# daovietanh190499/3D_Reconstruction

Hardware: AMD Instinct MI355X
Metric: image-pairs matched/sec (higher is better)
Workload: dtype f32 descriptors: int8 MFMA certified filter + f64 re-score; 1 GPU; C3/C4 all-pairs BF-L2 + ratio 0.75: 257 imgs x 4096 kpts x 256-d, exact f32-input semantics (oracle.match.bf_match_exact, bit for bit); pairs=32896, api=dist.match_all_pairs_sharded(exact=True), match_mode=exact-float, parallelism=pairs/1

## Files before the change

### 3d_reconstruction_amd/csrc/match.hip

```cpp
#include "common.h"
#include "fp6_sched.h"
#include <climits>
#include <cstdlib>

namespace sfmhip {

typedef int i32x4 __attribute__((ext_vector_type(4)));
typedef int i32x16 __attribute__((ext_vector_type(16)));

constexpr int kJB = 128;

template <int D>
__device__ __forceinline__ int swz_off(int r, int c) {
    constexpr int CPR = D / 16;
    constexpr int RPB = 256 / D;
    return r * D + ((c ^ ((r / RPB) % CPR)) << 4);
}

__device__ __forceinline__ int max3i(int a, int b, int c) {
    int r;
    asm("v_max3_i32 %0, %1, %2, %3" : "=v"(r) : "v"(a), "v"(b), "v"(c));
    return r;
}
__device__ __forceinline__ int med3i(int a, int b, int c) {
    int r;
    asm("v_med3_i32 %0, %1, %2, %3" : "=v"(r) : "v"(a), "v"(b), "v"(c));
    return r;
}

__global__ void quantize_kernel(const float* __restrict__ in, int64_t total, int d, int m_pad,
                                const int32_t* __restrict__ nk, int mode, int8_t* __restrict__ out) {
    const int64_t n4 = total >> 2;
    for (int64_t q = (int64_t)blockIdx.x * blockDim.x + threadIdx.x; q < n4;
         q += (int64_t)gridDim.x * blockDim.x) {
        const int64_t e = q << 2;
        const int64_t row = e / d;
        const int img = (int)(row / m_pad);
        const int r = (int)(row % m_pad);
        const float4 x = *reinterpret_cast<const float4*>(in + e);
        char4 o = make_char4(0, 0, 0, 0);
        if (r < nk[img]) {
            float v[4] = {x.x, x.y, x.z, x.w};
            int qv[4];
#pragma unroll
            for (int t = 0; t < 4; ++t) {
                if (mode == 0) {
                    float rr = fminf(fmaxf(__builtin_rintf(v[t]), 0.f), 255.f);
                    qv[t] = (int)rr - 128;
                } else {
                    float rr = __builtin_rintf(127.f * v[t]);
                    rr = fminf(fmaxf(rr, -127.f), 127.f);
                    qv[t] = (int)rr;
                }
            }
            o = make_char4((signed char)qv[0], (signed char)qv[1], (signed char)qv[2], (signed char)qv[3]);
        }
        *reinterpret_cast<char4*>(out + e) = o;
    }
}

__global__ void prepare_kernel(const int8_t* __restrict__ desc, int n_rows, int m_pad, int d,
                               const int32_t* __restrict__ nk, int32_t* __restrict__ norms,
                               int32_t* __restrict__ keys) {
    const int row = blockIdx.x * blockDim.x + threadIdx.x;
    if (row >= n_rows) return;
    const int img = row / m_pad, r = row % m_pad;
    const int8_t* p = desc + (size_t)row * d;
    int s = 0;
    for (int k = 0; k < d; k += 16) {
        const i32x4 v = *reinterpret_cast<const i32x4*>(p + k);
#pragma unroll
        for (int w = 0; w < 4; ++w) {
            const int x = v[w];
#pragma unroll
            for (int t = 0; t < 4; ++t) {
                const int q = (int)(signed char)((x >> (8 * t)) & 0xff);
                s += q * q;
            }
        }
    }
    norms[row] = s;
    const int low = 127 - (r & (kJB - 1));
    keys[row] = (r < nk[img]) ? (-s * 128 + low) : (INT_MIN + low);
}

__global__ void key_values_kernel(const int32_t* __restrict__ keys, int64_t n, int32_t* __restrict__ h,
                                  float* __restrict__ hf) {
    for (int64_t e = (int64_t)blockIdx.x * blockDim.x + threadIdx.x; e < n; e += (int64_t)gridDim.x * blockDim.x) {
        const int v = keys[e] >> 8;
        h[e] = v;
        if (hf) hf[e] = (float)v * 0.015625f;
    }
}

__device__ __forceinline__ int fp6_grid_index(float y, int* g) {
    const float t = fminf(fabsf(y), 60.f);
    int n, m;
    if (t < 16.f) { m = (int)__builtin_rintf(t); n = m; }
    else if (t < 32.f) { const int r = (int)__builtin_rintf(0.5f * t); m = 2 * r; n = r + 8; }
    else { const int r = (int)__builtin_rintf(0.25f * t); m = 4 * r; n = r + 16; }
    const bool neg = y < 0.f && m > 0;
    *g = neg ? -m : m;
    return n | (neg ? 32 : 0);
}
__global__ void quantize_fp6_kernel(const float* __restrict__ in, int64_t n_chunks, int d, int m_pad,
                                    const int32_t* __restrict__ nk, int8_t* __restrict__ g,
                                    uint8_t* __restrict__ code) {
    for (int64_t c = (int64_t)blockIdx.x * blockDim.x + threadIdx.x; c < n_chunks;
         c += (int64_t)gridDim.x * blockDim.x) {
        const int64_t e0 = c * 32, row = e0 / d;
        const int img = (int)(row / m_pad), r = (int)(row % m_pad);
        const bool valid = r < nk[img];
        unsigned gw[8], cw[8];
#pragma unroll
        for (int w = 0; w < 8; ++w) gw[w] = cw[w] = 0u;
        if (valid) {
#pragma unroll
            for (int q = 0; q < 8; ++q) {
                const float4 x = *reinterpret_cast<const float4*>(in + e0 + 4 * q);
                const float v[4] = {x.x, x.y, x.z, x.w};
                unsigned pk = 0u;
#pragma unroll
                for (int t = 0; t < 4; ++t) {
                    int gv;
                    const int cd = fp6_grid_index(127.f * v[t], &gv);
                    gw[q] |= (unsigned)(gv & 0xff) << (8 * t);
                    pk |= (unsigned)cd << (6 * t);
                }
#pragma unroll
                for (int t = 0; t < 3; ++t) {
                    const int byte = 3 * q + t;
                    cw[byte >> 2] |= ((pk >> (8 * t)) & 0xffu) << (8 * (byte & 3));
                }
            }
        }
        uint4* go = reinterpret_cast<uint4*>(g + e0);
        uint4* co = reinterpret_cast<uint4*>(code + e0);
        go[0] = make_uint4(gw[0], gw[1], gw[2], gw[3]);
        go[1] = make_uint4(gw[4], gw[5], gw[6], gw[7]);
        co[0] = make_uint4(cw[0], cw[1], cw[2], cw[3]);
        co[1] = make_uint4(cw[4], cw[5], cw[6], cw[7]);
    }
}

template <int D, int WAVES>
struct Stager {
    static constexpr int CPR = D / 16;
    static constexpr int RPB = 256 / D;
    static constexpr int TILE = kJB * D;
    static constexpr int NI = TILE / 1024;
    static constexpr int PER_WAVE = NI / WAVES;
    static constexpr int LDT = TILE / 16 / (64 * WAVES);
    static_assert(NI % WAVES == 0 && LDT >= 1, "block / workgroup mismatch");

    __device__ static void dma(const int8_t* src, const int32_t* ksrc, int8_t* dst, int32_t* kdst, int wave,
                               int lane) {
#pragma unroll
        for (int u = 0; u < PER_WAVE; ++u) {
            const int ins = wave * PER_WAVE + u;
            const int rows_per_ins = 1024 / D;
            const int r0 = ins * rows_per_ins;
            const int r = r0 + lane / CPR;
            const int c = (lane % CPR) ^ ((r / RPB) % CPR);
            __builtin_amdgcn_global_load_lds(
                (__attribute__((address_space(1))) void*)(src + (size_t)r * D + c * 16),
                (__attribute__((address_space(3))) void*)(dst + r0 * D), 16, 0, 0);
        }
        if (wave == WAVES - 1) {
#pragma unroll
            for (int u = 0; u < 2; ++u)
                __builtin_amdgcn_global_load_lds(
                    (__attribute__((address_space(1))) void*)(ksrc + u * 64 + lane),
                    (__attribute__((address_space(3))) void*)(kdst + u * 64), 4, 0, 0);
        }
    }
};

template <int MF> struct Mfma;
template <> struct Mfma<32> {
    using acc_t = i32x16;
    static constexpr int NREG = 16, KB = 32;
    __device__ static acc_t run(i32x4 a, i32x4 b, acc_t c) {
        return __builtin_amdgcn_mfma_i32_32x32x32_i8(a, b, c, 0, 0, 0);
    }
    __device__ static int row(int q, int grp) { return (q & 3) + 8 * (q >> 2) + 4 * grp; }
};
template <> struct Mfma<16> {
    using acc_t = i32x4;
    static constexpr int NREG = 4, KB = 64;
    __device__ static acc_t run(i32x4 a, i32x4 b, acc_t c) {
        return __builtin_amdgcn_mfma_i32_16x16x64_i8(a, b, c, 0, 0, 0);
    }
    __device__ static int row(int q, int grp) { return 4 * grp + q; }
};

struct CertArgs {
    const double* erow;
    const double* eimg;
    double inv_s;
    int force;
};
constexpr int kUndecidedBase = -3;
constexpr int kValueOnlyTiles = 4;
__device__ __forceinline__ int sqrt8_ceil(int d2) {
    const long long t = 64LL * d2;
    int u = (int)ceil(sqrt((double)t));
    while (u > 0 && (long long)(u - 1) * (u - 1) >= t) --u;
    while ((long long)u * u < t) ++u;
    return u;
}
template <typename OutT>
__device__ __forceinline__ int undecided_mark(int d2) {
    if constexpr (sizeof(OutT) == 2) return kUndecidedBase - sqrt8_ceil(d2);
    else return kUndecidedBase - d2;
}
template <typename OutT>
__device__ __forceinline__ double mark_sqrt_d2(int mark) {
    if constexpr (sizeof(OutT) == 2) return (double)(kUndecidedBase - mark) * 0.125;
    else return sqrt((double)(kUndecidedBase - mark));
}

__device__ __forceinline__ int certify(int d1lo, int d1hi, int d2lo, int d2hi, double E, double inv_s, double rn2,
                                       double rd2) {
    const double up = 1.0 + 0x1p-50, dn = 1.0 - 0x1p-50;
    const double s1l = sqrt((double)d1lo) * inv_s, s1h = sqrt((double)d1hi) * inv_s;
    const double s2l = sqrt((double)d2lo) * inv_s, s2h = sqrt((double)d2hi) * inv_s;
    const double a1 = fmax(s1l * dn - E * up, 0.0), b1 = (s1h + E) * up;
    const double a2 = fmax(s2l * dn - E * up, 0.0), b2 = (s2h + E) * up;
    const double wl = 1.0 - 1e-12, wh = 1.0 + 1e-12;
    const double lo1 = a1 * a1 * wl, hi1 = b1 * b1 * wh, lo2 = a2 * a2 * wl, hi2 = b2 * b2 * wh;
    if (rd2 * lo1 >= rn2 * hi2) return 0;
    if (hi1 < lo2 && rd2 * hi1 < rn2 * lo2) return 1;
    return -1;
}

template <int D, int MF, int NS, int VG, typename OutT>
__device__ __forceinline__ void value_only_tail(const int (&w1)[NS], const int (&w2)[NS], const int (&wr)[NS],
                                                const int8_t* __restrict__ desc, const int8_t* __restrict__ bdesc,
                                                const int32_t* __restrict__ bkeys, const int32_t* __restrict__ norms,
                                                int a, int b, int m_pad, int na_rows, int ibase, int grp, int lr,
                                                int lane, long long rn2, long long rd2, OutT* __restrict__ out_m,
                                                const CertArgs& ca) {
    constexpr int NG = 64 / MF;
    int v1 = INT_MIN, v2 = INT_MIN, loc = 0;
#pragma unroll
    for (int s = 0; s < NS; ++s) {
        int a1 = w1[s], a2 = w2[s], al = wr[s] * NG + grp;
#pragma unroll
        for (int off = MF; off < 64; off <<= 1) {
            const int o1 = __shfl_xor(a1, off), o2 = __shfl_xor(a2, off), ol = __shfl_xor(al, off);
            const bool mine = a1 > o1 || (a1 == o1 && al < ol);
            a2 = max3i(min(a1, o1), a2, o2);
            al = mine ? al : ol;
            a1 = max(a1, o1);
        }
        if (s == grp) { v1 = a1; v2 = a2; loc = al; }
    }
    const int i = ibase + grp * MF + lr;
    int res = -1, na = 0, du1 = 0, hidx = -1;
    double E = 0.0;
    bool survivor = false;
    if (i < na_rows) {
        na = norms[(size_t)a * m_pad + i];
        du1 = na - 2 * v1;
        const int du2ub = na - 2 * v2;
        E = ca.erow[(size_t)a * m_pad + i] + ca.eimg[b];
        if (ca.force)
            res = undecided_mark<OutT>(min(du2ub, D * 255 * 255));
        else
            survivor = certify(max(du1 - 1, 0), du1, max(du1 - 1, 0), du2ub, E, ca.inv_s, (double)rn2,
                               (double)rd2) != 0;
    }
    constexpr int NC = 4 * VG;
    constexpr int LPC = (64 / NC) < (D / 16) ? (64 / NC) : (D / 16);
    constexpr int BPL = D / LPC;
    const int c = min(lane / LPC, NC - 1), part = lane % LPC;
    unsigned long long bal = __ballot(survivor);
    while (bal) {
        const int l = __builtin_ctzll(bal);
        bal &= bal - 1;
        const int ri = __shfl(i, l), rv = __shfl(v1, l), rl = __shfl(loc, l);
        const int j0 = (rl / NG) * VG * MF + 4 * (rl % NG);
        const int j = j0 + (c >> 2) * MF + (c & 3);
        const int8_t* pa = desc + ((size_t)a * m_pad + ri) * D + part * BPL;
        const int8_t* pb = bdesc + (size_t)j * D + part * BPL;
        int dot = 0;
#pragma unroll
        for (int w = 0; w < BPL / 16; ++w) {
            const i32x4 x = *reinterpret_cast<const i32x4*>(pa + 16 * w);
            const i32x4 y = *reinterpret_cast<const i32x4*>(pb + 16 * w);
#pragma unroll
            for (int e = 0; e < 4; ++e) dot = __builtin_amdgcn_sdot4(x[e], y[e], dot, false);
        }
#pragma unroll
        for (int off = 1; off < LPC; off <<= 1) dot += __shfl_xor(dot, off);
        const int u = dot + bkeys[j];
        const bool hit = lane < NC * LPC && part == 0 && u == rv;
        const unsigned long long hb = __ballot(hit);
        int x = u == rv ? INT_MIN : u;
#pragma unroll
        for (int off = LPC; off < 64; off <<= 1) x = max(x, __shfl_xor(x, off));
        if (lane == l) {
            const bool one = __popcll(hb) == 1;
            v2 = max(v2, one ? x : rv);
            if (one) {
                const int hc = __builtin_ctzll(hb) / LPC;
                hidx = j0 + (hc >> 2) * MF + (hc & 3);
            }
        }
    }
    if (survivor) {
        const int du2 = na - 2 * v2;
        const int v = certify(max(du1 - 1, 0), du1, max(du2 - 1, 0), du2, E, ca.inv_s, (double)rn2, (double)rd2);
        res = v == 0 ? -1 : (v > 0 && hidx >= 0) ? hidx : undecided_mark<OutT>(du2);
    }
    if (i < m_pad) out_m[i] = (OutT)res;
}

template <int D, int MF, int NS, int WAVES, bool CERT = false, typename OutT = int32_t, int VG = 0>
__global__ __launch_bounds__(64 * WAVES, 2) void match_kernel(
    const int8_t* __restrict__ desc, const int32_t* __restrict__ norms,
    const int32_t* __restrict__ keys, const int32_t* __restrict__ nk, int m_pad,
    const int32_t* __restrict__ pairs, int n_iblk, int nwg, long long rn2, long long rd2,
    OutT* __restrict__ m0, int32_t* __restrict__ dist1, int32_t* __restrict__ dist2, CertArgs ca) {
    using S = Stager<D, WAVES>;
    using M = Mfma<MF>;
    using acc_t = typename M::acc_t;
    constexpr int KK = D / M::KB;
    constexpr int CPK = M::KB / 16;
    constexpr int NG = 64 / MF;
    constexpr int TILE = S::TILE;
    constexpr int NT = 64 * WAVES;
    constexpr int IW = MF * NS;
    constexpr int IB = IW * WAVES;
    constexpr int JT = kJB / MF;
    static_assert(NS % NG == 0 || NG % NS == 0, "output lane mapping");
    constexpr bool VO = VG > 0;
    static_assert(!VO || (CERT && M::NREG == 4 && NS == NG && JT % VG == 0), "value-only form: 16x16 tiles, NS == NG");

    __shared__ __attribute__((aligned(16))) int8_t lds[2 * TILE + 2 * kJB * 4];

    const int wg = xcd_remap(blockIdx.x, nwg);
    const int pair = wg / n_iblk, ib = wg % n_iblk;
    const int a = pairs[2 * pair], b = pairs[2 * pair + 1];
    const int na_rows = nk[a], nb_rows = nk[b];
    const int tid = threadIdx.x, lane = tid & 63;
    const int wave = __builtin_amdgcn_readfirstlane(tid >> 6);
    const int grp = lane / MF, lr = lane % MF;
    const int ibase = ib * IB + wave * IW;
    OutT* out_m = m0 + (size_t)pair * m_pad;

    if (ib * IB >= na_rows || nb_rows < 2) {
        const int iend = min(ib * IB + IB, m_pad);
        for (int i = ib * IB + tid; i < iend; i += NT) {
            out_m[i] = -1;
            if (dist1) dist1[(size_t)pair * m_pad + i] = -1;
            if (dist2) dist2[(size_t)pair * m_pad + i] = -1;
        }
        return;
    }

    const int8_t* bdesc = desc + (size_t)b * m_pad * D;
    const int32_t* bkeys = keys + (size_t)b * m_pad;
    const int nblk = (nb_rows + kJB - 1) / kJB;
    int32_t* kbase = reinterpret_cast<int32_t*>(lds + 2 * TILE);

    S::dma(bdesc, bkeys, lds, kbase, wave, lane);

    i32x4 bq[NS][KK];
#pragma unroll
    for (int s = 0; s < NS; ++s) {
        const int i = min(ibase + s * MF + lr, m_pad - 1);
        const int8_t* rp = desc + ((size_t)a * m_pad + i) * D + grp * 16;
#pragma unroll
        for (int kk = 0; kk < KK; ++kk) bq[s][kk] = *reinterpret_cast<const i32x4*>(rp + kk * M::KB);
    }

    int g1k[NS], g1i[NS], g2k[NS], g1w[NS], g1b[NS];
#pragma unroll
    for (int s = 0; s < NS; ++s) { g1k[s] = INT_MIN; g1i[s] = 0; g1w[s] = 127; g1b[s] = 0; g2k[s] = INT_MIN; }
    int w1[NS], w2[NS], wr[NS];
#pragma unroll
    for (int s = 0; s < NS; ++s) { w1[s] = INT_MIN; w2[s] = INT_MIN; wr[s] = 0; }

    __syncthreads();

    for (int blk = 0; blk < nblk; ++blk) {
        const int cur = blk & 1;
        if (blk + 1 < nblk)
            S::dma(bdesc + (size_t)(blk + 1) * TILE, bkeys + (blk + 1) * kJB, lds + (cur ^ 1) * TILE,
                   kbase + (cur ^ 1) * kJB, wave, lane);
        const int8_t* tl = lds + cur * TILE;
        const int32_t* kl = kbase + cur * kJB;
        if constexpr (VO) {
            int rm[NS];
#pragma unroll
            for (int jt = 0; jt < JT; ++jt) {
                if (jt % VG == 0) {
#pragma unroll
                    for (int s = 0; s < NS; ++s) rm[s] = INT_MIN;
                }
                const i32x4 hv = *reinterpret_cast<const i32x4*>(kl + jt * MF + M::row(0, grp));
                acc_t acc[NS];
#pragma unroll
                for (int s = 0; s < NS; ++s) acc[s] = hv;
                const int r = jt * MF + lr;
#pragma unroll
                for (int kk = 0; kk < KK; ++kk) {
                    const i32x4 av = *reinterpret_cast<const i32x4*>(tl + swz_off<D>(r, kk * CPK + grp));
#pragma unroll
                    for (int s = 0; s < NS; ++s) acc[s] = M::run(av, bq[s][kk], acc[s]);
                }
#pragma unroll
                for (int s = 0; s < NS; ++s) {
                    rm[s] = max(max(rm[s], acc[s][0]), acc[s][1]);
                    rm[s] = max(max(rm[s], acc[s][2]), acc[s][3]);
                }
                if (jt % VG == VG - 1) {
                    const int rid = blk * (JT / VG) + jt / VG;
#pragma unroll
                    for (int s = 0; s < NS; ++s) {
                        wr[s] = rm[s] > w1[s] ? rid : wr[s];
                        w2[s] = med3i(w1[s], w2[s], rm[s]);
                        w1[s] = max(w1[s], rm[s]);
                    }
                }
            }
            __syncthreads();
            continue;
        }
        int t1[NS], t2[NS];
#pragma unroll
        for (int s = 0; s < NS; ++s) { t1[s] = INT_MIN; t2[s] = INT_MIN; }
#pragma unroll
        for (int jt = 0; jt < JT; ++jt) {
            acc_t acc[NS];
#pragma unroll
            for (int s = 0; s < NS; ++s) acc[s] = acc_t{0};
            const int r = jt * MF + lr;
#pragma unroll
            for (int kk = 0; kk < KK; ++kk) {
                const i32x4 av = *reinterpret_cast<const i32x4*>(tl + swz_off<D>(r, kk * CPK + grp));
#pragma unroll
                for (int s = 0; s < NS; ++s) acc[s] = M::run(av, bq[s][kk], acc[s]);
            }
#pragma unroll
            for (int g = 0; g < M::NREG / 4; ++g) {
                const i32x4 kv = *reinterpret_cast<const i32x4*>(kl + jt * MF + M::row(4 * g, grp));
#pragma unroll
                for (int e = 0; e < 4; e += 2) {
#pragma unroll
                    for (int s = 0; s < NS; ++s) {
                        const int ka = acc[s][4 * g + e] * 256 + kv[e];
                        const int kb = acc[s][4 * g + e + 1] * 256 + kv[e + 1];
                        const int m = med3i(t1[s], ka, kb);
                        t1[s] = max3i(t1[s], ka, kb);
                        t2[s] = max(t2[s], m);
                    }
                }
            }
        }
#pragma unroll
        for (int s = 0; s < NS; ++s) {
            if constexpr (D <= 128) {
                const int k1 = t1[s] >> 7, k2 = t2[s] >> 7;
                const bool up = k1 > g1k[s];
                g2k[s] = max3i(min(g1k[s], k1), g2k[s], k2);
                g1w[s] = up ? t1[s] : g1w[s];
                g1b[s] = up ? blk : g1b[s];
                g1k[s] = max(g1k[s], k1);
            } else {
                const int k1 = t1[s] >> 7, k2 = t2[s] >> 7, ix = blk * kJB + 127 - (t1[s] & 127);
                if (k1 > g1k[s]) { g2k[s] = max(g1k[s], k2); g1k[s] = k1; g1i[s] = ix; }
                else             { g2k[s] = max(g2k[s], k1); }
            }
        }
        __syncthreads();
    }

    if constexpr (VO) {
        value_only_tail<D, MF, NS, VG, OutT>(w1, w2, wr, desc, bdesc, bkeys, norms, a, b, m_pad, na_rows, ibase, grp, lr,
                                             lane, rn2, rd2, out_m, ca);
        return;
    }
    if constexpr (D <= 128) {
#pragma unroll
        for (int s = 0; s < NS; ++s) g1i[s] = g1b[s] * kJB + 127 - (g1w[s] & 127);
    }
#pragma unroll
    for (int s = 0; s < NS; ++s) {
#pragma unroll
        for (int off = MF; off < 64; off <<= 1) {
            const int ok = __shfl_xor(g1k[s], off), oi = __shfl_xor(g1i[s], off), o2 = __shfl_xor(g2k[s], off);
            const bool mine = (g1k[s] > ok) || (g1k[s] == ok && g1i[s] < oi);
            const int n2 = mine ? max(g2k[s], ok) : max(o2, g1k[s]);
            if (!mine) { g1k[s] = ok; g1i[s] = oi; }
            g2k[s] = n2;
        }
    }
#pragma unroll
    for (int s = 0; s < NS; ++s) {
        if (s % NG != grp % NS) continue;
        const int i = ibase + s * MF + lr;
        if (i >= m_pad) continue;
        int res = -1, d1 = -1, d2 = -1;
        if (i < na_rows) {
            const int na = norms[(size_t)a * m_pad + i];
            d1 = na - g1k[s];
            d2 = na - g2k[s];
            if (CERT) {
                const int v = ca.force ? -1
                                       : certify(d1, d1, d2, d2, ca.erow[(size_t)a * m_pad + i] + ca.eimg[b], ca.inv_s,
                                                 (double)rn2, (double)rd2);
                res = v > 0 ? g1i[s] : (v == 0 ? -1 : undecided_mark<OutT>(d2));
            } else if (rd2 * (long long)d1 < rn2 * (long long)d2) {
                res = g1i[s];
            }
        }
        out_m[i] = (OutT)res;
        if (dist1) dist1[(size_t)pair * m_pad + i] = d1;
        if (dist2) dist2[(size_t)pair * m_pad + i] = d2;
    }
}

typedef int i32x2 __attribute__((ext_vector_type(2)));
typedef int i32x8 __attribute__((ext_vector_type(8)));
typedef float f32x4 __attribute__((ext_vector_type(4)));

__global__ void pack_fp6_kernel(const uint8_t* __restrict__ code, int64_t n_chunks, int d,
                                uint8_t* __restrict__ dense) {
    const int spr = d / 32;
    for (int64_t c = (int64_t)blockIdx.x * blockDim.x + threadIdx.x; c < n_chunks;
         c += (int64_t)gridDim.x * blockDim.x) {
        const int64_t row = c / spr;
        const int s = (int)(c % spr);
        const uint4 lo = *reinterpret_cast<const uint4*>(code + c * 32);
        const uint2 hi = *reinterpret_cast<const uint2*>(code + c * 32 + 16);
        uint8_t* rp = dense + row * (3 * d / 4);
        *reinterpret_cast<uint4*>(rp + 16 * s) = lo;
        *reinterpret_cast<uint2*>(rp + d / 2 + 8 * s) = hi;
    }
}

template <int D, int WAVES>
struct DenseStager {
    static constexpr int ROW = 3 * D / 4, LB = D / 2, HB = D / 4;
    static constexpr int LO = kJB * LB, TILE = kJB * ROW;
    static constexpr int CPR = LB / 16, RPB = 256 / LB;
    static constexpr int UPR = HB / 16, RPH = 256 / HB;
    static constexpr int NLO = LO / 1024 / WAVES, NHI = (TILE - LO) / 1024 / WAVES;
    static_assert(NLO * WAVES * 1024 == LO && NHI * WAVES * 1024 == TILE - LO && NLO >= 1 && NHI >= 1,
                  "block / workgroup mismatch");
    static_assert(RPB * CPR == 16 && RPH * UPR == 16, "a 16-row tile covers every bank once");

    __device__ static int lo_sw(int r) { return ((((r & 15) + 4) >> 3) & 1) ^ ((r / RPB) % CPR); }
    __device__ static int hi_sw(int r) { return (r / RPH) % UPR; }
    __device__ static int lo_off(int r, int s) { return r * LB + ((s ^ lo_sw(r)) << 4); }
    __device__ static int hi_off(int r, int s) { return LO + r * HB + ((((s >> 1) ^ hi_sw(r)) << 4) | ((s & 1) << 3)); }

    struct Lanes {
        unsigned lo[NLO], hi[NHI], key;
    };
    __device__ static Lanes lanes(int wave, int lane) {
        Lanes l;
#pragma unroll
        for (int u = 0; u < NLO; ++u) {
            const int r = (wave * NLO + u) * (1024 / LB) + lane / CPR;
            l.lo[u] = (unsigned)(r * ROW + (((lane % CPR) ^ lo_sw(r)) << 4));
        }
#pragma unroll
        for (int u = 0; u < NHI; ++u) {
            const int r = (wave * NHI + u) * (1024 / HB) + lane / UPR;
            l.hi[u] = (unsigned)(r * ROW + LB + (((lane % UPR) ^ hi_sw(r)) << 4));
        }
        l.key = (unsigned)(lane * 4);
        return l;
    }

    __device__ static void dma(const uint8_t* src, const int32_t* ksrc, int8_t* dst, int32_t* kdst, int wave,
                               const Lanes& l) {
#pragma unroll
        for (int u = 0; u < NLO; ++u) {
            unsigned o = l.lo[u];
            asm volatile("" : "+v"(o));
            __builtin_amdgcn_global_load_lds((__attribute__((address_space(1))) void*)(src + o),
                                             (__attribute__((address_space(3))) void*)(dst + (wave * NLO + u) * 1024),
                                             16, 0, 0);
        }
#pragma unroll
        for (int u = 0; u < NHI; ++u) {
            unsigned o = l.hi[u];
            asm volatile("" : "+v"(o));
            __builtin_amdgcn_global_load_lds(
                (__attribute__((address_space(1))) void*)(src + o),
                (__attribute__((address_space(3))) void*)(dst + LO + (wave * NHI + u) * 1024), 16, 0, 0);
        }
        if (wave == WAVES - 1) {
#pragma unroll
            for (int u = 0; u < 2; ++u)
                __builtin_amdgcn_global_load_lds(
                    (__attribute__((address_space(1))) void*)(reinterpret_cast<const uint8_t*>(ksrc + u * 64) + l.key),
                    (__attribute__((address_space(3))) void*)(kdst + u * 64), 4, 0, 0);
        }
    }
};

__device__ __forceinline__ i32x2 lds_read_b64(const int8_t* p) {
    return *(const volatile __attribute__((address_space(3))) i32x2*)p;
}

struct Fp6Operand {
    i32x4 lo;
    i32x2 hi;
    __device__ i32x8 tuple() const { return i32x8{lo[0], lo[1], lo[2], lo[3], hi[0], hi[1], 0, 0}; }
};

constexpr int kFp6Tiles = 8;
constexpr int kFp6Waves = 4;

template <int D, typename OutT>
__global__ __launch_bounds__(64 * kFp6Waves, 2) void match_fp6_kernel(
    const uint8_t* __restrict__ dense, const int8_t* __restrict__ g, const int32_t* __restrict__ norms,
    const int32_t* __restrict__ h, const float* __restrict__ hf, const int32_t* __restrict__ nk, int m_pad,
    const int32_t* __restrict__ pairs, int n_iblk, int nwg, long long rn2, long long rd2,
    OutT* __restrict__ m0, CertArgs ca) {
    constexpr int MF = 16, NS = kFp6Tiles, WAVES = kFp6Waves, VG = kValueOnlyTiles;
    static_assert(D % 128 == 0, "one MFMA takes 128 elements of k");
    static_assert(NS % 4 == 0, "value_only_tail takes four query tiles at a time");
    using S = DenseStager<D, WAVES>;
    constexpr int KK = D / 128;
    using SC = Fp6Sched<KK, NS>;
    static_assert(kJB / MF == 2 * VG, "two ranges per block: the range maxima alternate between two sets");
    static_assert(SC::merge(VG * SC::MPT, 0) == -1, "a range's gaps hold the previous range's merge");
    static_assert(SC::merge_ready(), "a chain's merge starts behind its last maximum");
    constexpr int TILE = S::TILE;
    constexpr int NT = 64 * WAVES;
    constexpr int IW = MF * NS, IB = IW * WAVES;
    constexpr int JT = kJB / MF;
    constexpr int kScale = 0;
    constexpr float kLow = -262144.f;

    __shared__ __attribute__((aligned(16))) int8_t lds[2 * TILE + 2 * kJB * 4];

    const int wg = xcd_remap(blockIdx.x, nwg);
    const int pair = wg / n_iblk, ib = wg % n_iblk;
    const int a = pairs[2 * pair], b = pairs[2 * pair + 1];
    const int na_rows = nk[a], nb_rows = nk[b];
    const int tid = threadIdx.x, lane = tid & 63;
    const int wave = __builtin_amdgcn_readfirstlane(tid >> 6);
    const int grp = lane / MF, lr = lane % MF;
    const int ibase = ib * IB + wave * IW;
    OutT* out_m = m0 + (size_t)pair * m_pad;

    if (ib * IB >= na_rows || nb_rows < 2) {
        const int iend = min(ib * IB + IB, m_pad);
        for (int i = ib * IB + tid; i < iend; i += NT) out_m[i] = -1;
        return;
    }

    const uint8_t* bdense = dense + (size_t)b * m_pad * S::ROW;
    const int32_t* bhf = reinterpret_cast<const int32_t*>(hf) + (size_t)b * m_pad;
    const int nblk = (nb_rows + kJB - 1) / kJB;
    int32_t* kbase = reinterpret_cast<int32_t*>(lds + 2 * TILE);

    const typename S::Lanes dl = S::lanes(wave, lane);
    S::dma(bdense, bhf, lds, kbase, wave, dl);

    Fp6Operand bq[NS][KK];
#pragma unroll
    for (int s = 0; s < NS; ++s) {
        const int i = min(ibase + s * MF + lr, m_pad - 1);
        const uint8_t* rp = dense + ((size_t)a * m_pad + i) * S::ROW;
#pragma unroll
        for (int kk = 0; kk < KK; ++kk) {
            bq[s][kk].lo = *reinterpret_cast<const i32x4*>(rp + 16 * (kk * 4 + grp));
            bq[s][kk].hi = *reinterpret_cast<const i32x2*>(rp + S::LB + 8 * (kk * 4 + grp));
        }
    }
    int lo_b[KK], hi_b[KK];
#pragma unroll
    for (int kk = 0; kk < KK; ++kk) {
        lo_b[kk] = S::lo_off(lr, kk * 4 + grp);
        hi_b[kk] = S::hi_off(lr, kk * 4 + grp);
    }

    float w1[NS], w2[NS];
    int wr[NS];
    f32x4 acc[NS];
    float half[NS], rm[2][NS];
    bool up[NS];
    int rid_owed = 0;
#pragma unroll
    for (int s = 0; s < NS; ++s) {
        w1[s] = kLow; w2[s] = kLow; wr[s] = 0;
        acc[s] = f32x4{kLow, kLow, kLow, kLow};
        half[s] = rm[0][s] = rm[1][s] = kLow;
        up[s] = false;
    }
    auto merge_step = [&](int c, int step, float m, int rid) {
        fp6_merge_step(step, m, rid, up[c], w1[c], w2[c], wr[c]);
    };

    __syncthreads();

    const uint8_t* bsrc = bdense;
    const int32_t* ksrc = bhf;
    for (int blk = 0; blk < nblk; ++blk) {
        const int cur = blk & 1;
        bsrc += TILE;
        ksrc += kJB;
        if (blk + 1 < nblk)
            S::dma(bsrc, ksrc, lds + (cur ^ 1) * TILE, kbase + (cur ^ 1) * kJB, wave, dl);
        const int8_t* tl = lds + cur * TILE;
        const float* kl = reinterpret_cast<const float*>(kbase + cur * kJB);
        Fp6Operand av;
        av.lo = *reinterpret_cast<const i32x4*>(tl + lo_b[0]);
        av.hi = lds_read_b64(tl + hi_b[0]);
        f32x4 hv = *reinterpret_cast<const f32x4*>(kl + 4 * grp);
#pragma unroll
        for (int jt = 0; jt < JT; ++jt) {
            const int R = jt / VG, tt = jt % VG;
            f32x4 hv_n = hv;
#pragma unroll
            for (int kk = 0; kk < KK; ++kk) {
                Fp6Operand av_n = av;
                __builtin_amdgcn_sched_barrier(0);
#pragma unroll
                for (int s = 0; s < NS; ++s) {
                    acc[s] = __builtin_amdgcn_mfma_scale_f32_16x16x128_f8f6f4(av.tuple(), bq[s][kk].tuple(),
                                                                              kk == 0 ? hv : acc[s], 2, 2, 0, kScale, 0,
                                                                              kScale);
                    __builtin_amdgcn_sched_barrier(0);
                    if (s == 0) {
                        if (kk + 1 < KK) {
                            av_n.lo = *reinterpret_cast<const i32x4*>(tl + lo_b[kk + 1] + jt * MF * S::LB);
                            av_n.hi = lds_read_b64(tl + hi_b[kk + 1] + jt * MF * S::HB);
                        } else if (jt + 1 < JT) {
                            av_n.lo = *reinterpret_cast<const i32x4*>(tl + lo_b[0] + (jt + 1) * MF * S::LB);
                            av_n.hi = lds_read_b64(tl + hi_b[0] + (jt + 1) * MF * S::HB);
                            hv_n = *reinterpret_cast<const f32x4*>(kl + (jt + 1) * MF + 4 * grp);
                        }
                        __builtin_amdgcn_sched_barrier(0);
                    }
                    const int gp = kk * NS + s;
                    if (const int c = SC::chain(gp, 0); c < NS) {
                        const int of = tt - SC::back(gp, 0);
                        const float from = of < 0 ? rm[R ^ 1][c] : of == 0 ? kLow : rm[R][c];
                        half[c] = __builtin_fmaxf(__builtin_fmaxf(from, acc[c][0]), acc[c][1]);
                    }
                    if (const int c = SC::chain(gp, 1); c < NS)
                        rm[tt == 0 && SC::back(gp, 1) ? R ^ 1 : R][c] =
                            __builtin_fmaxf(__builtin_fmaxf(half[c], acc[c][2]), acc[c][3]);
#pragma unroll
                    for (int j = 0; j < SC::kBudget; ++j)
                        if (const int k = SC::merge(tt * SC::MPT + gp, j); k >= 0) {
                            __builtin_amdgcn_sched_barrier(0);
                            merge_step(SC::merge_chain(k), SC::merge_step(k), rm[R ^ 1][SC::merge_chain(k)], rid_owed);
                        }
                    __builtin_amdgcn_sched_barrier(0);
                }
                av = av_n;
            }
            hv = hv_n;
            if (tt == VG - 1) rid_owed = blk * (JT / VG) + R;
        }
        __syncthreads();
    }
#pragma unroll
    for (int s = SC::kOwedFirst; s < NS; ++s)
        half[s] = __builtin_fmaxf(__builtin_fmaxf(rm[1][s], acc[s][0]), acc[s][1]);
#pragma unroll
    for (int s = SC::kOwedSecond; s < NS; ++s)
        rm[1][s] = __builtin_fmaxf(__builtin_fmaxf(half[s], acc[s][2]), acc[s][3]);
#pragma unroll
    for (int s = 0; s < NS; ++s)
#pragma unroll
        for (int step = 0; step < 4; ++step) merge_step(s, step, rm[1][s], rid_owed);

#pragma unroll
    for (int q = 0; q < NS / 4; ++q) {
        int v1[4], v2[4], vr[4];
#pragma unroll
        for (int s = 0; s < 4; ++s) {
            v1[s] = (int)(64.f * w1[4 * q + s]);
            v2[s] = (int)(64.f * w2[4 * q + s]);
            vr[s] = wr[4 * q + s];
        }
        value_only_tail<D, MF, 4, VG, OutT>(v1, v2, vr, g, g + (size_t)b * m_pad * D, h + (size_t)b * m_pad, norms, a, b,
                                            m_pad, na_rows, ibase + q * 4 * MF, grp, lr, lane, rn2, rd2, out_m, ca);
    }
}

__global__ void mutual_kernel(int32_t* __restrict__ m0, int32_t* __restrict__ m1, int P, int m_pad) {
    const int64_t total = (int64_t)P * m_pad;
    for (int64_t e = (int64_t)blockIdx.x * blockDim.x + threadIdx.x; e < total;
         e += (int64_t)gridDim.x * blockDim.x) {
        const int64_t base = (e / m_pad) * m_pad;
        const int i = (int)(e - base);
        const int j0 = m0[e];
        const int j1 = m1[e];
        const bool keep0 = j0 >= 0 && m1[base + j0] == i;
        const bool keep1 = j1 >= 0 && m0[base + j1] == i;
        if (j0 >= 0 && !keep0) m0[e] = -1;
        if (j1 >= 0 && !keep1) m1[e] = -1;
    }
}

constexpr int kVqObsPerBlock = 16;
constexpr int kVqCodesPerChunk = 32;

__global__ __launch_bounds__(256) void vq_kernel(const double* __restrict__ obs, int64_t n_obs,
                                                 const double* __restrict__ code, int n_codes, int d,
                                                 int32_t* __restrict__ codes, double* __restrict__ dist) {
    extern __shared__ double smem[];
    double* sobs = smem;
    double* scode = smem + kVqObsPerBlock * d;
    const int ld = d + 1;
    const int64_t o0 = (int64_t)blockIdx.x * kVqObsPerBlock;
    for (int t = threadIdx.x; t < kVqObsPerBlock * d; t += blockDim.x) {
        const int64_t o = o0 + t / d;
        sobs[t] = (o < n_obs) ? obs[o * d + (t % d)] : 0.0;
    }
    const int lo = threadIdx.x >> 4, l16 = threadIdx.x & 15;
    const double* x = sobs + lo * d;
    double best = __builtin_inf();
    int bidx = INT_MAX;
    for (int c0 = 0; c0 < n_codes; c0 += kVqCodesPerChunk) {
        const int nc = min(kVqCodesPerChunk, n_codes - c0);
        __syncthreads();
        for (int t = threadIdx.x; t < nc * d; t += blockDim.x) {
            const int r = t / d;
            scode[r * ld + (t - r * d)] = code[(size_t)(c0 + r) * d + (t - r * d)];
        }
        __syncthreads();
        double acc[2] = {0.0, 0.0};
        for (int k = 0; k < d; ++k) {
            const double xv = x[k];
#pragma unroll
            for (int j = 0; j < 2; ++j) {
                const int r = l16 + 16 * j;
                const double df = xv - scode[r * ld + k];
                acc[j] = __builtin_fma(df, df, acc[j]);
            }
        }
#pragma unroll
        for (int j = 0; j < 2; ++j) {
            const int r = l16 + 16 * j;
            if (r < nc && acc[j] < best) { best = acc[j]; bidx = c0 + r; }
        }
    }
#pragma unroll
    for (int off = 8; off >= 1; off >>= 1) {
        const double ob = __shfl_xor(best, off, 16);
        const int oi = __shfl_xor(bidx, off, 16);
        if (ob < best || (ob == best && oi < bidx)) { best = ob; bidx = oi; }
    }
    const int64_t o = o0 + lo;
    if (l16 == 0 && o < n_obs) {
        codes[o] = bidx;
        dist[o] = sqrt(best);
    }
}

typedef double v4d __attribute__((ext_vector_type(4)));
constexpr int kVqmWaves = 8;
constexpr int kVqmObsPerWave = 32;
constexpr int kVqmTile = kVqmWaves * kVqmObsPerWave;

template <int DP, bool FULL>
__global__ __launch_bounds__(kVqmWaves * 64) void vq_mfma_kernel(
    const double* __restrict__ obs, int64_t n_obs, const double* __restrict__ code, int n_codes, int d,
    int codes_per_pass, int32_t* __restrict__ codes, double* __restrict__ dist) {
    constexpr int LD = DP + 4;
    constexpr int KS = DP / 4;
    extern __shared__ double smem[];
    double* sc = smem;
    double* sn = smem + (size_t)codes_per_pass * LD;
    const int lane = threadIdx.x & 63, wave = threadIdx.x >> 6;
    const int r16 = lane & 15, kq = lane >> 4;
    const int64_t n_tiles = (n_obs + kVqmTile - 1) / kVqmTile;
    for (int c0 = 0; c0 < n_codes; c0 += codes_per_pass) {
        const int nc = min(codes_per_pass, n_codes - c0);
        const int ncb = (nc + 15) >> 4;
        const bool first = c0 == 0, last = c0 + codes_per_pass >= n_codes;
        __syncthreads();
        for (int t = threadIdx.x; t < ncb * 16 * DP; t += blockDim.x) {
            const int r = t / DP, k = t - r * DP;
            sc[r * LD + k] = (r < nc && (FULL || k < d)) ? code[(size_t)(c0 + r) * d + k] : 0.0;
        }
        __syncthreads();
        for (int r = threadIdx.x; r < ncb * 16; r += blockDim.x) {
            double s = 0.0;
            for (int k = 0; k < DP; ++k) s = __builtin_fma(sc[r * LD + k], sc[r * LD + k], s);
            sn[r] = r < nc ? s : __builtin_inf();
        }
        __syncthreads();
        for (int64_t t = blockIdx.x; t < n_tiles; t += gridDim.x) {
            const int64_t ob = t * kVqmTile + wave * kVqmObsPerWave;
            double a[2][KS];
#pragma unroll
            for (int h = 0; h < 2; ++h) {
                const int64_t o = ob + 16 * h + r16;
                const double* xp = obs + o * d;
#pragma unroll
                for (int s = 0; s < KS; ++s) {
                    const int k = 4 * s + kq;
                    a[h][s] = (o < n_obs && (FULL || k < d)) ? __builtin_nontemporal_load(xp + k) : 0.0;
                }
            }
            double best[2][4];
            int bj[2][4];
#pragma unroll
            for (int h = 0; h < 2; ++h)
#pragma unroll
                for (int g = 0; g < 4; ++g) { best[h][g] = __builtin_inf(); bj[h][g] = INT_MAX; }
            auto epilogue = [&](const v4d& acc0, const v4d& acc1, int j) {
                const double cn = sn[j];
#pragma unroll
                for (int g = 0; g < 4; ++g) {
                    const double d0 = cn - 2.0 * acc0[g];
                    const double d1 = cn - 2.0 * acc1[g];
                    if (d0 < best[0][g]) { best[0][g] = d0; bj[0][g] = c0 + j; }
                    if (d1 < best[1][g]) { best[1][g] = d1; bj[1][g] = c0 + j; }
                }
            };
            for (int cb = 0; cb < ncb; ++cb) {
                const int j = cb * 16 + r16;
                const double* bp = sc + j * LD + kq;
                v4d acc0 = {0.0, 0.0, 0.0, 0.0}, acc1 = {0.0, 0.0, 0.0, 0.0};
#pragma unroll
                for (int s = 0; s < KS; ++s) {
                    const double b = bp[4 * s];
                    acc0 = __builtin_amdgcn_mfma_f64_16x16x4f64(a[0][s], b, acc0, 0, 0, 0);
                    acc1 = __builtin_amdgcn_mfma_f64_16x16x4f64(a[1][s], b, acc1, 0, 0, 0);
                }
                epilogue(acc0, acc1, j);
            }
#pragma unroll
            for (int h = 0; h < 2; ++h) {
                int win = 0;
#pragma unroll
                for (int g = 0; g < 4; ++g) {
                    double bv = best[h][g];
                    int bi = bj[h][g];
#pragma unroll
                    for (int off = 8; off >= 1; off >>= 1) {
                        const double ov = __shfl_xor(bv, off, 16);
                        const int oi = __shfl_xor(bi, off, 16);
                        if (ov < bv || (ov == bv && oi < bi)) { bv = ov; bi = oi; }
                    }
                    const int64_t o = ob + 16 * h + kq + 4 * g;
                    if (!first && o < n_obs) {
                        const double prev = dist[o];
                        if (!(bv < prev)) { bv = prev; bi = codes[o]; }
                    }
                    if (!last && r16 == 0 && o < n_obs) {
                        codes[o] = bi;
                        dist[o] = bv;
                    }
                    const int w = __shfl(bi, (r16 & 3) * 16);
                    if ((r16 >> 2) == g) win = w;
                }
                if (last) {
                    const int64_t o = ob + 16 * h + r16;
                    const double* cp = code + (size_t)win * d;
                    double part = 0.0;
#pragma unroll
                    for (int s = 0; s < KS; ++s) {
                        const int k = 4 * s + kq;
                        const double df = a[h][s] - ((o < n_obs && (FULL || k < d)) ? cp[k] : 0.0);
                        part = __builtin_fma(df, df, part);
                    }
                    part += __shfl_xor(part, 16);
                    part += __shfl_xor(part, 32);
                    if (kq == 0 && o < n_obs) {
                        codes[o] = win;
                        dist[o] = sqrt(part);
                    }
                }
            }
        }
    }
}


typedef float f32x4 __attribute__((ext_vector_type(4)));
__device__ __forceinline__ double vq_eps_abs(int DP, double xn, double cmax) {
    return 0x1p-126 * (2.0 * sqrt((double)DP) * (cmax + xn) + 2.0 * DP + 4.0) * 1.01;
}
typedef double f64x2 __attribute__((ext_vector_type(2)));
typedef _Float16 f16x8 __attribute__((ext_vector_type(8)));
constexpr int kVqhWaves = 8;
__device__ __forceinline__ double vq_eps16(int DP, double xn, double cmax) {
    const double u = 0x1p-24;
    return 1.01 * (2.0 * xn * cmax * (0x1.8p-21 + 2.02 * DP * u + 4.0 * u) + 4.0 * u * cmax * cmax +
                   0x1p-24 * sqrt((double)DP) * (xn + cmax) + 2.0 * DP * 0x1p-48) +
           vq_eps_abs(DP, xn, cmax);
}
__device__ __forceinline__ int vqh_k(int j, int e, int q) { return 16 * (j & 7) + 4 * q + 2 * (j >> 3) + e; }
__device__ __forceinline__ double vqh_xor8(double v) {
    const int lo = __builtin_amdgcn_mov_dpp((int)__double2loint(v), 0x128, 0xF, 0xF, false);
    const int hi = __builtin_amdgcn_mov_dpp((int)__double2hiint(v), 0x128, 0xF, 0xF, false);
    return __hiloint2double(hi, lo);
}
template <int PROBE>
__global__ __launch_bounds__(kVqhWaves * 64) void vq_f16s_kernel(const double* __restrict__ obs, int64_t n_obs,
                                                                  const double* __restrict__ code, int n_codes,
                                                                  int32_t* __restrict__ codes,
                                                                  double* __restrict__ dist,
                                                                  unsigned* __restrict__ amb,
                                                                  unsigned* __restrict__ namb) {
    constexpr int DP = 128, KB = 4, KS = 32;
    extern __shared__ f32x4 smh[];
    const int ncb = (n_codes + 15) >> 4;
    const int ncp = (ncb + 1) & ~1;
    f16x8* sc = reinterpret_cast<f16x8*>(smh);
    float* sn = reinterpret_cast<float*>(smh + ncp * KB * 2 * 64);
    __shared__ unsigned s_cmax, s_big;
    const int lane = threadIdx.x & 63, wave = __builtin_amdgcn_readfirstlane(threadIdx.x >> 6);
    const int r16 = lane & 15, kq = lane >> 4;
    const bool b3 = (lane >> 3) & 1;
    if (threadIdx.x == 0) { s_cmax = 0u; s_big = 0u; }
    __syncthreads();
    for (int t = threadIdx.x; t < ncp * KB * 64; t += blockDim.x) {
        const int ln = t & 63, kb = (t >> 6) % KB, cb = t / (KB * 64);
        const int j = cb * 16 + (ln & 15);
        f16x8 hi, lo;
        bool big = false;
#pragma unroll
        for (int e = 0; e < 8; ++e) {
            const double v = j < n_codes ? code[(size_t)j * DP + vqh_k(4 * kb + (e >> 1), e & 1, ln >> 4)] : 0.0;
            big |= !(fabs(v) < 32768.0);
            const _Float16 h = (_Float16)(float)v;
            hi[e] = h;
            lo[e] = (_Float16)(float)(v - (double)h);
        }
        if (big) s_big = 1u;
        sc[((cb * KB + kb) * 2 + 0) * 64 + ln] = hi;
        sc[((cb * KB + kb) * 2 + 1) * 64 + ln] = lo;
    }
    for (int r = threadIdx.x; r < ncp * 16; r += blockDim.x) {
        double q = 0.0;
        if (r < n_codes)
            for (int k = 0; k < DP; ++k) q = __builtin_fma(code[(size_t)r * DP + k], code[(size_t)r * DP + k], q);
        sn[r] = r < n_codes ? (float)q : __builtin_inff();
        if (r < n_codes) atomicMax(&s_cmax, __float_as_uint((float)sqrt(q) * 1.001f));
    }
    __syncthreads();
    const double cmax = (double)__uint_as_float(s_cmax);
    const bool book_big = s_big != 0u;
    const int64_t n_units = (n_obs + 15) >> 4;
    const int64_t ustep = (int64_t)gridDim.x * kVqhWaves;
    f64x2 nx[KS / 2];
    auto fetch = [&](int64_t un) {
#pragma unroll
        for (int j = 0; j < KS / 2; ++j) {
            const f64x2* xp = reinterpret_cast<const f64x2*>(
                                  obs + min(un * 16 + (lane & 7) + 8 * (j >> 3), n_obs - 1) * DP) +
                              8 * (j & 7) + 2 * kq + b3;
            nx[j] = PROBE == 1 ? f64x2{(double)(lane + un) * 0x1p-10, (double)j * 0x1p-10}
                               : __builtin_nontemporal_load(xp);
        }
    };
    fetch(min((int64_t)blockIdx.x * kVqhWaves + wave, n_units - 1));
    for (int64_t un = (int64_t)blockIdx.x * kVqhWaves + wave; un < n_units; un += ustep) {
        const int64_t o = un * 16 + r16;
        double x[KS];
#pragma unroll
        for (int m = 0; m < 8; ++m) {
            const f64x2 a0 = nx[m], a1 = nx[8 + m];
            const double s0 = vqh_xor8(b3 ? a0.x : a1.x), s1 = vqh_xor8(b3 ? a0.y : a1.y);
            x[2 * m] = b3 ? s0 : a0.x;
            x[2 * m + 1] = b3 ? s1 : a0.y;
            x[16 + 2 * m] = b3 ? a1.x : s0;
            x[16 + 2 * m + 1] = b3 ? a1.y : s1;
        }
        fetch(min(un + ustep, n_units - 1));
        double xn = 0.0;
        bool big = book_big;
#pragma unroll
        for (int s = 0; s < KS; ++s) {
            xn = __builtin_fma(x[s], x[s], xn);
            big |= !(fabs(x[s]) < 32768.0);
        }
        xn += __shfl_xor(xn, 16);
        xn += __shfl_xor(xn, 32);
        f16x8 ah[KB], al[KB];
#pragma unroll
        for (int b = 0; b < KB; ++b)
#pragma unroll
            for (int e = 0; e < 8; ++e) {
                const _Float16 h = (_Float16)(float)x[8 * b + e];
                ah[b][e] = h;
                al[b][e] = (_Float16)(float)(x[8 * b + e] - (double)h);
            }
        float b1[4], b2[4];
        int i1[4];
#pragma unroll
        for (int g = 0; g < 4; ++g) { b1[g] = b2[g] = __builtin_inff(); i1[g] = INT_MAX; }
        auto take = [&](int g, float dd, int j) {
            const bool l = dd < b1[g];
            b2[g] = l ? b1[g] : fminf(dd, b2[g]);
            i1[g] = l ? j : i1[g];
            b1[g] = l ? dd : b1[g];
        };
        for (int cb = 0; cb < (PROBE == 4 ? 0 : ncb); cb += 2) {
            const f16x8* bp = sc + cb * KB * 2 * 64 + lane;
            f32x4 m0 = {0.f, 0.f, 0.f, 0.f}, m1 = m0, c0 = m0, c1 = m0;
#pragma unroll
            for (int b = 0; b < KB; ++b) {
                const f16x8 c0h = bp[(b * 2 + 0) * 64], c0l = bp[(b * 2 + 1) * 64];
                const f16x8 c1h = bp[((KB + b) * 2 + 0) * 64], c1l = bp[((KB + b) * 2 + 1) * 64];
                m0 = __builtin_amdgcn_mfma_f32_16x16x32_f16(ah[b], c0h, m0, 0, 0, 0);
                m1 = __builtin_amdgcn_mfma_f32_16x16x32_f16(ah[b], c1h, m1, 0, 0, 0);
                c0 = __builtin_amdgcn_mfma_f32_16x16x32_f16(ah[b], c0l, c0, 0, 0, 0);
                c1 = __builtin_amdgcn_mfma_f32_16x16x32_f16(ah[b], c1l, c1, 0, 0, 0);
                c0 = __builtin_amdgcn_mfma_f32_16x16x32_f16(al[b], c0h, c0, 0, 0, 0);
                c1 = __builtin_amdgcn_mfma_f32_16x16x32_f16(al[b], c1h, c1, 0, 0, 0);
            }
            const int j0 = cb * 16 + r16;
            const float cn0 = sn[j0], cn1 = sn[j0 + 16];
#pragma unroll
            for (int g = 0; g < 4; ++g) {
                take(g, cn0 - 2.f * (m0[g] + c0[g]), j0);
                take(g, cn1 - 2.f * (m1[g] + c1[g]), j0 + 16);
            }
        }
        const double eps_row = vq_eps16(DP, sqrt(xn), cmax);
        int win[4];
#pragma unroll
        for (int g = 0; g < 4; ++g) {
            float v1 = b1[g], v2 = b2[g];
            int x1 = i1[g];
#pragma unroll
            for (int off = 8; off >= 1; off >>= 1) {
                const float o1 = __shfl_xor(v1, off, 16), o2 = __shfl_xor(v2, off, 16);
                const int ox = __shfl_xor(x1, off, 16);
                const bool t = o1 < v1 || (o1 == v1 && ox < x1);
                v2 = t ? fminf(v1, o2) : fminf(o1, v2);
                v1 = t ? o1 : v1;
                x1 = t ? ox : x1;
            }
            const double eps = __shfl(eps_row, 4 * kq + g);
            win[g] = PROBE == 4 ? (4 * kq + g) % n_codes : ((double)v2 - (double)v1 > 2.0 * eps) ? x1 : -1;
        }
        int w = -1;
#pragma unroll
        for (int g = 0; g < 4; ++g) {
            const int t = __shfl(win[g], (r16 >> 2) << 4);
            if ((r16 & 3) == g) w = t;
        }
        const bool rbig = __shfl_xor((int)big, 16) | __shfl_xor((int)big, 32) | __shfl_xor((int)big, 48) | big;
        if (rbig) w = -1;
        const f64x2* cp = reinterpret_cast<const f64x2*>(code + (size_t)max(w, 0) * DP) + 2 * kq;
        double part = 0.0;
#pragma unroll
        for (int b = 0; b < KB; ++b) {
#pragma unroll
            for (int t = 0; t < 4; ++t) {
                const int j = 4 * b + t;
                const f64x2 c = PROBE == 2 ? f64x2{x[2 * j + 1], x[2 * j]} : cp[8 * (j & 7) + (j >> 3)];
                const double d0 = x[2 * j] - c.x, d1 = x[2 * j + 1] - c.y;
                part = __builtin_fma(d0, d0, part);
                part = __builtin_fma(d1, d1, part);
            }
            __builtin_amdgcn_sched_barrier(0);
        }
        part += __shfl_xor(part, 16);
        part += __shfl_xor(part, 32);
        if (kq == 0 && o < n_obs) {
            if (w >= 0) {
                codes[o] = w;
                dist[o] = sqrt(part);
            } else {
                amb[atomicAdd(namb, 1u)] = (unsigned)o;
            }
        }
    }
}

__global__ __launch_bounds__(256) void vq_exact_kernel(const double* __restrict__ obs, const double* __restrict__ code,
                                                       int n_codes, int d, const unsigned* __restrict__ amb,
                                                       const unsigned* __restrict__ namb, int32_t* __restrict__ codes,
                                                       double* __restrict__ dist) {
    const int lane = threadIdx.x & 63, cg = lane >> 4, k16 = lane & 15;
    const unsigned n = *namb;
    for (unsigned e = blockIdx.x * 4 + __builtin_amdgcn_readfirstlane(threadIdx.x >> 6); e < n; e += gridDim.x * 4) {
        const int64_t o = amb[e];
        const double* xp = obs + o * d;
        double best = __builtin_inf();
        int bi = INT_MAX;
        for (int j0 = 0; j0 < n_codes; j0 += 4) {
            const int j = j0 + cg;
            const double* cp = code + (size_t)min(j, n_codes - 1) * d;
            double q = 0.0;
            for (int k0 = 8 * k16; k0 < d; k0 += 128) {
#pragma unroll
                for (int t = 0; t < 8; ++t) {
                    const int k = k0 + t;
                    if (k < d) {
                        const double df = xp[k] - cp[k];
                        q = __builtin_fma(df, df, q);
                    }
                }
            }
#pragma unroll
            for (int off = 8; off >= 1; off >>= 1) q += __shfl_xor(q, off, 16);
            if (j < n_codes && q < best) { best = q; bi = j; }
        }
#pragma unroll
        for (int off = 32; off >= 16; off >>= 1) {
            const double ob = __shfl_xor(best, off);
            const int oi = __shfl_xor(bi, off);
            if (ob < best || (ob == best && oi < bi)) { best = ob; bi = oi; }
        }
        if (lane == 0) {
            codes[o] = bi;
            dist[o] = sqrt(best);
        }
    }
}


__global__ __launch_bounds__(256) void desc_residual_kernel(const float* __restrict__ x, const int8_t* __restrict__ q,
                                                            int n_rows, int m_pad, int d, const int32_t* __restrict__ nk,
                                                            int mode, double* __restrict__ erow,
                                                            unsigned long long* __restrict__ eimg) {
    const int lane = threadIdx.x & 63;
    const int row = blockIdx.x * 4 + (threadIdx.x >> 6);
    if (row >= n_rows) return;
    const int img = row / m_pad, r = row % m_pad;
    if (r >= nk[img]) {
        if (lane == 0) erow[row] = 0.0;
        return;
    }
    const float* xr = x + (size_t)row * d;
    const int8_t* qr = q + (size_t)row * d;
    double s2 = 0.0, x2 = 0.0, v2 = 0.0;
    bool finite = true;
    for (int k = lane; k < d; k += 64) {
        const float xf = xr[k];
        const double xv = (double)xf;
        const double v = mode == 0 ? (double)((int)qr[k] + 128) : (double)qr[k] / 127.0;
        const double dl = xv - v;
        s2 = __builtin_fma(dl, dl, s2);
        x2 = __builtin_fma(xv, xv, x2);
        v2 = __builtin_fma(v, v, v2);
        finite = finite && __builtin_isfinite(xf);
    }
#pragma unroll
    for (int off = 32; off >= 1; off >>= 1) {
        s2 += __shfl_xor(s2, off);
        x2 += __shfl_xor(x2, off);
        v2 += __shfl_xor(v2, off);
    }
    const bool all_finite = __all(finite);
    if (lane == 0) {
        const double e = all_finite ? sqrt(s2) * (1.0 + 0x1p-40) + 0x1p-50 * (sqrt(x2) + sqrt(v2)) * (1.0 + 0x1p-40)
                                    : __builtin_inf();
        erow[row] = e;
        atomicMax(eimg + img, (unsigned long long)__double_as_longlong(e));
    }
}

constexpr int kResolveCap = 512;
#ifdef SFMHIP_RESOLVE_PROF
__device__ unsigned long long g_rprof[16];
#endif
template <int D, typename OutT>
__device__ __forceinline__ void resolve_row(int64_t e, int mark, const int8_t* __restrict__ q,
                                            const float* __restrict__ x, const int32_t* __restrict__ nk, int m_pad,
                                            const int32_t* __restrict__ pairs, const double* __restrict__ erow,
                                            const double* __restrict__ eimg, double s, double rn2, double rd2,
                                            OutT* __restrict__ m0, unsigned* __restrict__ n_resolved, float* sxa,
                                            int* sqa, int* scand, int lane) {
    constexpr int W4 = D / 4;
    const int pair = (int)(e / m_pad), i = (int)(e % m_pad);
    const int a = pairs[2 * pair], b = pairs[2 * pair + 1], nb = nk[b];
    const size_t arow = (size_t)a * m_pad + i;
    for (int k = lane; k < D; k += 64) sxa[k] = x[arow * D + k];
    for (int w = lane; w < W4; w += 64) sqa[w] = reinterpret_cast<const int*>(q + arow * D)[w];
    __builtin_amdgcn_fence(__ATOMIC_RELEASE, "wavefront");
    __builtin_amdgcn_wave_barrier();
    __builtin_amdgcn_fence(__ATOMIC_ACQUIRE, "wavefront");
    int na = 0;
    for (int w = lane; w < W4; w += 64) na = __builtin_amdgcn_sdot4(sqa[w], sqa[w], na, false);
#pragma unroll
    for (int off = 32; off >= 1; off >>= 1) na += __shfl_xor(na, off);
    const double se = (erow[arow] + eimg[b]) * s * (1.0 + 1e-12);
    const double bq = (se + (mark_sqrt_d2<OutT>(mark) + se) * (1.0 + 1e-12)) * (1.0 + 1e-12);
    const double tq = floor(bq * bq) + 1.0;
    int ncand = 0;
    for (int j0 = 0; j0 < nb; j0 += 64) {
        const int j = j0 + lane;
        bool in = false;
        if (j < nb) {
            const int4* qb = reinterpret_cast<const int4*>(q + ((size_t)b * m_pad + j) * D);
            int dot = 0, nbn = 0;
#pragma unroll 4
            for (int w4 = 0; w4 < W4 / 4; ++w4) {
                const int4 t = qb[w4];
                const int4 u = reinterpret_cast<const int4*>(sqa)[w4];
                dot = __builtin_amdgcn_sdot4(t.x, u.x, dot, false);
                dot = __builtin_amdgcn_sdot4(t.y, u.y, dot, false);
                dot = __builtin_amdgcn_sdot4(t.z, u.z, dot, false);
                dot = __builtin_amdgcn_sdot4(t.w, u.w, dot, false);
                nbn = __builtin_amdgcn_sdot4(t.x, t.x, nbn, false);
                nbn = __builtin_amdgcn_sdot4(t.y, t.y, nbn, false);
                nbn = __builtin_amdgcn_sdot4(t.z, t.z, nbn, false);
                nbn = __builtin_amdgcn_sdot4(t.w, t.w, nbn, false);
            }
            in = (double)((long long)na + nbn - 2LL * dot) <= tq;
        }
        const unsigned long long cb = __ballot(in);
        const int pos = ncand + __popcll(cb & ((1ull << lane) - 1ull));
        if (in && pos < kResolveCap) scand[pos] = j;
        ncand += __popcll(cb);
    }
    __builtin_amdgcn_fence(__ATOMIC_RELEASE, "wavefront");
    __builtin_amdgcn_wave_barrier();
    __builtin_amdgcn_fence(__ATOMIC_ACQUIRE, "wavefront");
    const bool every = ncand > kResolveCap;
    const int nc = every ? nb : ncand;
    double v1 = __builtin_inf(), v2 = __builtin_inf();
    int j1 = INT_MAX;
    for (int t = lane; t < nc; t += 64) {
        const int j = every ? t : scand[t];
        const float4* xb = reinterpret_cast<const float4*>(x + ((size_t)b * m_pad + j) * D);
        double acc = 0.0;
        for (int k4 = 0; k4 < D / 4; ++k4) {
            const float4 xv = xb[k4];
            double df;
            df = (double)sxa[4 * k4] - (double)xv.x;
            acc = acc + df * df;
            df = (double)sxa[4 * k4 + 1] - (double)xv.y;
            acc = acc + df * df;
            df = (double)sxa[4 * k4 + 2] - (double)xv.z;
            acc = acc + df * df;
            df = (double)sxa[4 * k4 + 3] - (double)xv.w;
            acc = acc + df * df;
        }
        if (acc < v1) { v2 = v1; v1 = acc; j1 = j; }
        else if (acc < v2) v2 = acc;
    }
#pragma unroll
    for (int off = 32; off >= 1; off >>= 1) {
        const double o1 = __shfl_xor(v1, off), o2 = __shfl_xor(v2, off);
        const int oj = __shfl_xor(j1, off);
        const bool mine = v1 < o1 || (v1 == o1 && j1 < oj);
        const double n2 = mine ? fmin(v2, o1) : fmin(o2, v1);
        if (!mine) { v1 = o1; j1 = oj; }
        v2 = n2;
    }
    const double p1 = rd2 * v1, e1 = __builtin_fma(rd2, v1, -p1);
    const double p2 = rn2 * v2, e2 = __builtin_fma(rn2, v2, -p2);
    const bool acc_ok = p1 < p2 || (p1 == p2 && e1 < e2);
    if (lane == 0) {
        m0[e] = (OutT)(acc_ok ? j1 : -1);
        if (n_resolved) atomicAdd(n_resolved, 1u);
    }
    __builtin_amdgcn_wave_barrier();
}

template <int D, typename OutT>
__global__ __launch_bounds__(256) void match_resolve_kernel(const int8_t* __restrict__ q, const float* __restrict__ x,
                                                            const int32_t* __restrict__ nk, int m_pad,
                                                            const int32_t* __restrict__ pairs, int P,
                                                            const double* __restrict__ erow,
                                                            const double* __restrict__ eimg, double s, double rn2,
                                                            double rd2, OutT* __restrict__ m0,
                                                            unsigned* __restrict__ n_resolved,
                                                            const unsigned* __restrict__ overflow = nullptr) {
    if (overflow && *overflow == 0u) return;
    constexpr int W4 = D / 4;
    __shared__ float sxa[4][D];
    __shared__ __attribute__((aligned(16))) int sqa[4][W4];
    __shared__ int scand[4][kResolveCap];
    const int lane = threadIdx.x & 63, wave = threadIdx.x >> 6;
    const int64_t total = (int64_t)P * m_pad;
    const int64_t nchunk = (total + 63) >> 6;
    for (int64_t c = (int64_t)blockIdx.x * 4 + wave; c < nchunk; c += (int64_t)gridDim.x * 4) {
        const int64_t e0 = c << 6;
        const int v = (e0 + lane < total) ? (int)m0[e0 + lane] : -1;
        unsigned long long bal = __ballot(v <= kUndecidedBase);
        while (bal) {
            const int l = __builtin_ctzll(bal);
            bal &= bal - 1;
            resolve_row<D, OutT>(e0 + l, __shfl(v, l), q, x, nk, m_pad, pairs, erow, eimg, s, rn2, rd2, m0, n_resolved,
                           sxa[wave], sqa[wave], scand[wave], lane);
        }
    }
}

constexpr int kResolveBucket = 4096;
template <typename OutT>
__global__ __launch_bounds__(256) void resolve_collect_kernel(const OutT* __restrict__ m0, int64_t total, int m_pad,
                                                              const int32_t* __restrict__ pairs,
                                                              unsigned* __restrict__ cnt, int64_t* __restrict__ list,
                                                              unsigned* __restrict__ overflow) {
    auto take = [&](int64_t e) {
        const int b = pairs[2 * (int)(e / m_pad) + 1];
        const unsigned slot = atomicAdd(cnt + b, 1u);
        if (slot < (unsigned)kResolveBucket) list[(size_t)b * kResolveBucket + slot] = e;
        else atomicOr(overflow, 1u);
    };
    constexpr int PER = 16 / sizeof(OutT);
    const int64_t n4 = total / PER;
    const int4* m4 = reinterpret_cast<const int4*>(m0);
    for (int64_t e4 = (int64_t)blockIdx.x * blockDim.x + threadIdx.x; e4 < n4; e4 += (int64_t)gridDim.x * blockDim.x) {
        const int4 v = m4[e4];
        if constexpr (sizeof(OutT) == 2) {
            const unsigned w[4] = {(unsigned)v.x, (unsigned)v.y, (unsigned)v.z, (unsigned)v.w};
            bool any = false;
#pragma unroll
            for (int h = 0; h < 4; ++h) {
                any |= (short)(w[h] & 0xFFFFu) <= kUndecidedBase;
                any |= (short)(w[h] >> 16) <= kUndecidedBase;
            }
            if (!any) continue;
#pragma unroll
            for (int h = 0; h < 4; ++h) {
                if ((short)(w[h] & 0xFFFFu) <= kUndecidedBase) take(PER * e4 + 2 * h);
                if ((short)(w[h] >> 16) <= kUndecidedBase) take(PER * e4 + 2 * h + 1);
            }
        } else {
            if (min(min(v.x, v.y), min(v.z, v.w)) > kUndecidedBase) continue;
            if (v.x <= kUndecidedBase) take(4 * e4);
            if (v.y <= kUndecidedBase) take(4 * e4 + 1);
            if (v.z <= kUndecidedBase) take(4 * e4 + 2);
            if (v.w <= kUndecidedBase) take(4 * e4 + 3);
        }
    }
}

constexpr int kResolveRows = 16;
__global__ __launch_bounds__(1024) void resolve_offsets_kernel(
    const unsigned* __restrict__ cnt, int n_img, unsigned* __restrict__ off,
    unsigned* __restrict__ okey , int* __restrict__ oimg,
    unsigned* __restrict__ xr, int* __restrict__ items ,
    unsigned* __restrict__ ir , const unsigned* __restrict__ overflow) {
    __shared__ unsigned sr[1024], sk[1024];
    __shared__ unsigned sxs[9], sks[9];
    if (*overflow != 0u) return;
    const int tid = threadIdx.x;
    const int cap = n_img * (kResolveBucket / kResolveRows + 1);
    int ps[9];
    ps[0] = 0;
#pragma unroll
    for (int x = 0; x < 8; ++x) ps[x + 1] = ps[x] + (x < n_img ? (n_img - x + 7) / 8 : 0);
    unsigned carry_r = 0, carry_k = 0;
    for (int base = 0; base < n_img; base += 1024) {
        const int p = base + tid;
        int b = -1;
        unsigned cb = 0, ni = 0;
        if (p < n_img) {
            int x = 0;
#pragma unroll
            for (int y = 1; y < 8; ++y) x += (p >= ps[y]) ? 1 : 0;
            b = x + 8 * (p - ps[x]);
            cb = min(cnt[b], (unsigned)kResolveBucket);
            ni = (cb + kResolveRows - 1) / kResolveRows;
        }
        sr[tid] = cb;
        sk[tid] = ni;
        __syncthreads();
        for (int d = 1; d < 1024; d <<= 1) {
            const unsigned vr = tid >= d ? sr[tid - d] : 0u, vk = tid >= d ? sk[tid - d] : 0u;
            __syncthreads();
            sr[tid] += vr;
            sk[tid] += vk;
            __syncthreads();
        }
        const unsigned run = carry_r + sr[tid] - cb, k0 = carry_k + sk[tid] - ni;
        if (b >= 0) {
            off[b] = run;
            okey[p] = run;
            oimg[p] = b;
#pragma unroll
            for (int x = 0; x < 8; ++x)
                if (p == ps[x]) {
                    sxs[x] = run;
                    sks[x] = k0;
                }
            for (unsigned i = 0; i < ni; ++i) {
                items[k0 + i] = (int)(run + i * kResolveRows);
                items[cap + k0 + i] = (int)min((unsigned)kResolveRows, cb - i * kResolveRows);
                items[2 * cap + k0 + i] = b;
            }
        }
        carry_r += sr[1023];
        carry_k += sk[1023];
        __syncthreads();
    }
    if (tid < 9) {
        if (tid == 8 || ps[tid] >= n_img) {
            sxs[tid] = carry_r;
            sks[tid] = carry_k;
        }
    }
    __syncthreads();
    if (tid < 8) {
        xr[tid] = sxs[tid];
        xr[8 + tid] = sxs[tid + 1] - sxs[tid];
        ir[tid] = sks[tid];
        ir[8 + tid] = sks[tid + 1] - sks[tid];
    }
    if (tid == 0) okey[n_img] = carry_r;
}
__global__ __launch_bounds__(256) void resolve_flatten_kernel(const unsigned* __restrict__ okey,
                                                              const int* __restrict__ oimg, int n_img,
                                                              const int64_t* __restrict__ list,
                                                              int64_t* __restrict__ flat,
                                                              const unsigned* __restrict__ overflow) {
    if (*overflow != 0u) return;
    const unsigned total = okey[n_img];
    for (unsigned t = blockIdx.x * blockDim.x + threadIdx.x; t < total; t += gridDim.x * blockDim.x) {
        int lo = 0, hi = n_img - 1;
        while (lo < hi) {
            const int mid = (lo + hi + 1) >> 1;
            if (okey[mid] <= t) lo = mid;
            else hi = mid - 1;
        }
        flat[t] = list[(size_t)oimg[lo] * kResolveBucket + (t - okey[lo])];
    }
}

template <int D, typename OutT>
__global__ __launch_bounds__(256) void match_resolve_batched_kernel(
    const int8_t* __restrict__ q , const int32_t* __restrict__ norms,
    const float* __restrict__ x, const int32_t* __restrict__ nk, int m_pad,
    const int32_t* __restrict__ pairs, int n_img, const double* __restrict__ erow, const double* __restrict__ eimg,
    double s, double rn2, double rd2, OutT* __restrict__ m0, unsigned* __restrict__ n_resolved,
    const int64_t* __restrict__ flat, const int* __restrict__ items, const unsigned* __restrict__ ir,
    const unsigned* __restrict__ overflow) {
    constexpr int W4 = D / 4, R = kResolveRows;
    __shared__ __attribute__((aligned(16))) int sqa[R][W4];
    __shared__ float sxa[R][D];
    __shared__ int scand[R][kResolveCap];
    __shared__ int sncand[R], sna[R], sccd[R];
    __shared__ double stq[R];
    __shared__ int64_t se_[R];
    if (*overflow != 0u) return;
    const int tid = threadIdx.x, lane = tid & 63, wave = tid >> 6;
    const int cap = n_img * (kResolveBucket / kResolveRows + 1);
    const int xcd = blockIdx.x % 8, nx = (gridDim.x + 7 - xcd) / 8;
    const unsigned ib = ir[xcd], in = ir[8 + xcd];
    for (unsigned k = blockIdx.x / 8; k < in; k += nx) {
        const int f0 = items[ib + k], nr = items[cap + ib + k], b = items[2 * cap + ib + k];
        const int nb = nk[b];
        for (int t = tid; t < nr * W4; t += 256) {
            const int r = t / W4, w = t % W4;
            const int64_t e = flat[f0 + r];
            const size_t arow = (size_t)pairs[2 * (int)(e / m_pad)] * m_pad + (int)(e % m_pad);
            sqa[r][w] = reinterpret_cast<const int*>(q + arow * D)[w];
        }
        for (int t = tid; t < nr * D; t += 256) {
            const int r = t / D, kk = t % D;
            const int64_t e = flat[f0 + r];
            const size_t arow = (size_t)pairs[2 * (int)(e / m_pad)] * m_pad + (int)(e % m_pad);
            sxa[r][kk] = x[arow * D + kk];
        }
        if (tid < R) sncand[tid] = 0;
        __syncthreads();
        for (int r = wave; r < nr; r += 4) {
            int na = 0;
            for (int w = lane; w < W4; w += 64) na = __builtin_amdgcn_sdot4(sqa[r][w], sqa[r][w], na, false);
#pragma unroll
            for (int off = 32; off >= 1; off >>= 1) na += __shfl_xor(na, off);
            if (lane == 0) {
                const int64_t e = flat[f0 + r];
                const size_t arow = (size_t)pairs[2 * (int)(e / m_pad)] * m_pad + (int)(e % m_pad);
                const double se = (erow[arow] + eimg[b]) * s * (1.0 + 1e-12);
                const double bq = (se + (mark_sqrt_d2<OutT>((int)m0[e]) + se) * (1.0 + 1e-12)) * (1.0 + 1e-12);
                stq[r] = floor(bq * bq) + 1.0;
                sna[r] = na;
                sccd[r] = norms[arow] - na;
                se_[r] = e;
            }
        }
        __syncthreads();
        {
            using M16 = Mfma<16>;
            constexpr int KK = D / M16::KB;
            const int lr = lane & 15, grp = lane >> 4;
            i32x4 bqv[KK];
#pragma unroll
            for (int kk = 0; kk < KK; ++kk) bqv[kk] = *reinterpret_cast<const i32x4*>(&sqa[lr][kk * 16 + grp * 4]);
            const bool live = lr < nr;
            const long long na_r = live ? (long long)sna[lr] - sccd[lr] : 0;
            const double tq_r = live ? stq[lr] : -1.0;
            const size_t bbase = (size_t)b * m_pad;
            constexpr int TG = 4;
            for (int jg = wave * 16; jg < nb; jg += 64 * TG) {
                i32x4 av[TG][KK], nv[TG];
#pragma unroll
                for (int t = 0; t < TG; ++t) {
                    const int j0 = min(jg + 64 * t, m_pad - 16);
                    const int8_t* rp = q + (bbase + j0 + lr) * D + grp * 16;
#pragma unroll
                    for (int kk = 0; kk < KK; ++kk) av[t][kk] = *reinterpret_cast<const i32x4*>(rp + kk * M16::KB);
                    nv[t] = *reinterpret_cast<const i32x4*>(norms + bbase + j0 + 4 * grp);
                }
#pragma unroll
                for (int t = 0; t < TG; ++t) {
                    const int j0 = jg + 64 * t;
                    i32x4 acc = {0, 0, 0, 0};
#pragma unroll
                    for (int kk = 0; kk < KK; ++kk) acc = M16::run(av[t][kk], bqv[kk], acc);
#pragma unroll
                    for (int e = 0; e < 4; ++e) {
                        const int j = j0 + 4 * grp + e;
                        if (live && j < nb && (double)(na_r + nv[t][e] - 2LL * acc[e]) <= tq_r) {
                            const int pos = atomicAdd(&sncand[lr], 1);
                            if (pos < kResolveCap) scand[lr][pos] = j;
                        }
                    }
                }
            }
        }
        __syncthreads();
        for (int r = wave; r < nr; r += 4) {
            const int ncand = sncand[r];
            const bool every = ncand > kResolveCap;
#ifdef SFMHIP_RESOLVE_PROF
            if (lane == 0) {
                atomicAdd(&g_rprof[0], 1ull);
                atomicAdd(&g_rprof[1], (unsigned long long)ncand);
                if (every) atomicAdd(&g_rprof[2], 1ull);
                atomicMax(&g_rprof[3], (unsigned long long)ncand);
                atomicAdd(&g_rprof[4 + min(ncand / 64, 11)], 1ull);
            }
#endif
            const int nc = every ? nb : ncand;
            double v1 = __builtin_inf(), v2 = __builtin_inf();
            int j1 = INT_MAX;
            for (int t = lane; t < nc; t += 64) {
                const int j = every ? t : scand[r][t];
                const float4* xb = reinterpret_cast<const float4*>(x + ((size_t)b * m_pad + j) * D);
                double acc = 0.0;
                for (int k4 = 0; k4 < D / 4; ++k4) {
                    const float4 xv = xb[k4];
                    double df;
                    df = (double)sxa[r][4 * k4] - (double)xv.x;
                    acc = acc + df * df;
                    df = (double)sxa[r][4 * k4 + 1] - (double)xv.y;
                    acc = acc + df * df;
                    df = (double)sxa[r][4 * k4 + 2] - (double)xv.z;
                    acc = acc + df * df;
                    df = (double)sxa[r][4 * k4 + 3] - (double)xv.w;
                    acc = acc + df * df;
                }
                if (acc < v1 || (acc == v1 && j < j1)) { v2 = v1; v1 = acc; j1 = j; }
                else if (acc < v2) v2 = acc;
            }
#pragma unroll
            for (int off = 32; off >= 1; off >>= 1) {
                const double o1 = __shfl_xor(v1, off), o2 = __shfl_xor(v2, off);
                const int oj = __shfl_xor(j1, off);
                const bool mine = v1 < o1 || (v1 == o1 && j1 < oj);
                const double n2 = mine ? fmin(v2, o1) : fmin(o2, v1);
                if (!mine) { v1 = o1; j1 = oj; }
                v2 = n2;
            }
            const double p1 = rd2 * v1, e1 = __builtin_fma(rd2, v1, -p1);
            const double p2 = rn2 * v2, e2 = __builtin_fma(rn2, v2, -p2);
            const bool acc_ok = p1 < p2 || (p1 == p2 && e1 < e2);
            if (lane == 0) {
                m0[se_[r]] = (OutT)(acc_ok ? j1 : -1);
                if (n_resolved) atomicAdd(n_resolved, 1u);
            }
        }
        __syncthreads();
    }
}

}

using namespace sfmhip;

#ifdef SFMHIP_RESOLVE_PROF
extern "C" int sfmhip_debug_resolve_prof(unsigned long long* out) {
    return hipMemcpyFromSymbol(out, HIP_SYMBOL(sfmhip::g_rprof), sizeof(unsigned long long) * 16) == hipSuccess ? 0 : -2;
}
#endif

extern "C" int sfmhip_desc_quantize(const float* in, int n_img, int m_pad, int d,
                                    const int32_t* n_kpts, int mode, int8_t* out, void* stream) {
    SFMHIP_REQUIRE(in && out && n_kpts, "sfmhip_desc_quantize: null pointer");
    SFMHIP_REQUIRE(n_img > 0 && m_pad > 0 && d > 0 && d % 4 == 0, "sfmhip_desc_quantize: bad shape");
    SFMHIP_REQUIRE(mode == 0 || mode == 1, "sfmhip_desc_quantize: mode must be 0 or 1");
    const int64_t total = (int64_t)n_img * m_pad * d;
    const int64_t n4 = total / 4;
    const int grid = (int)std::min<int64_t>((n4 + 255) / 256, 4096);
    hipLaunchKernelGGL(quantize_kernel, dim3(grid), dim3(256), 0, as_stream(stream), in, total, d,
                       m_pad, n_kpts, mode, out);
    return check_launch("quantize_kernel");
}

extern "C" int sfmhip_desc_quantize_fp6(const float* in, int n_img, int m_pad, int d, const int32_t* n_kpts,
                                        int8_t* g, uint8_t* code, void* stream) {
    SFMHIP_REQUIRE(in && g && code && n_kpts, "sfmhip_desc_quantize_fp6: null pointer");
    SFMHIP_REQUIRE(n_img > 0 && m_pad > 0 && d > 0 && d % 32 == 0, "sfmhip_desc_quantize_fp6: bad shape");
    const int64_t n_chunks = (int64_t)n_img * m_pad * d / 32;
    const int grid = (int)std::min<int64_t>((n_chunks + 255) / 256, 4096);
    hipLaunchKernelGGL(quantize_fp6_kernel, dim3(grid), dim3(256), 0, as_stream(stream), in, n_chunks, d, m_pad,
                       n_kpts, g, code);
    return check_launch("quantize_fp6_kernel");
}

extern "C" int sfmhip_desc_pack_fp6(const uint8_t* code, int n_img, int m_pad, int d, uint8_t* dense, void* stream) {
    SFMHIP_REQUIRE(code && dense, "sfmhip_desc_pack_fp6: null pointer");
    SFMHIP_REQUIRE(n_img > 0 && m_pad > 0 && d > 0 && d % 64 == 0, "sfmhip_desc_pack_fp6: bad shape");
    const int64_t n_chunks = (int64_t)n_img * m_pad * d / 32;
    const int grid = (int)std::min<int64_t>((n_chunks + 255) / 256, 4096);
    hipLaunchKernelGGL(pack_fp6_kernel, dim3(grid), dim3(256), 0, as_stream(stream), code, n_chunks, d, dense);
    return check_launch("pack_fp6_kernel");
}

extern "C" int sfmhip_desc_prepare(const int8_t* desc, int n_img, int m_pad, int d,
                                   const int32_t* n_kpts, int32_t* norms, int32_t* keys, void* stream) {
    SFMHIP_REQUIRE(desc && n_kpts && norms && keys, "sfmhip_desc_prepare: null pointer");
    SFMHIP_REQUIRE(n_img > 0 && m_pad > 0 && d > 0 && d % 16 == 0, "sfmhip_desc_prepare: bad shape");
    const int rows = n_img * m_pad;
    hipLaunchKernelGGL(prepare_kernel, dim3(ceil_div(rows, 256)), dim3(256), 0, as_stream(stream),
                       desc, rows, m_pad, d, n_kpts, norms, keys);
    return check_launch("prepare_kernel");
}

__global__ void prepare_shifted_kernel(const int8_t* __restrict__ desc, int n_rows, int m_pad, int d,
                                       const int32_t* __restrict__ nk, int c, int8_t* __restrict__ out,
                                       int32_t* __restrict__ norms, int32_t* __restrict__ keys) {
    const int row = blockIdx.x * blockDim.x + threadIdx.x;
    if (row >= n_rows) return;
    const int img = row / m_pad, r = row % m_pad;
    const bool valid = r < nk[img];
    const int8_t* p = desc + (size_t)row * d;
    int8_t* o = out + (size_t)row * d;
    int s = 0, sum = 0;
    for (int k = 0; k < d; k += 16) {
        const i32x4 v = *reinterpret_cast<const i32x4*>(p + k);
        i32x4 w;
#pragma unroll
        for (int e = 0; e < 4; ++e) {
            const int x = v[e];
            unsigned packed = 0;
#pragma unroll
            for (int t = 0; t < 4; ++t) {
                const int q = (int)(signed char)((x >> (8 * t)) & 0xff);
                s += q * q;
                sum += q;
                packed |= (unsigned)((valid ? q + c : 0) & 0xff) << (8 * t);
            }
            w[e] = (int)packed;
        }
        *reinterpret_cast<i32x4*>(o + k) = w;
    }
    norms[row] = s + 2 * c * sum + 2 * c * c * d;
    const int low = 127 - (r & (kJB - 1));
    keys[row] = valid ? (-(s + 2 * c * sum) * 128 + low) : (INT_MIN + low);
}

extern "C" int sfmhip_desc_prepare_shifted(const int8_t* desc, int n_img, int m_pad, int d, const int32_t* n_kpts,
                                           int shift, int8_t* desc_shifted, int32_t* norms, int32_t* keys,
                                           void* stream) {
    SFMHIP_REQUIRE(desc && n_kpts && desc_shifted && norms && keys, "sfmhip_desc_prepare_shifted: null pointer");
    SFMHIP_REQUIRE(n_img > 0 && m_pad > 0 && d > 0 && d % 16 == 0 && d <= 256,
                   "sfmhip_desc_prepare_shifted: bad shape");
    SFMHIP_REQUIRE(shift >= 0 && shift <= 127, "sfmhip_desc_prepare_shifted: shift must be in [0, 127]");
    const int rows = n_img * m_pad;
    hipLaunchKernelGGL(prepare_shifted_kernel, dim3(ceil_div(rows, 256)), dim3(256), 0, as_stream(stream), desc,
                       rows, m_pad, d, n_kpts, shift, desc_shifted, norms, keys);
    return check_launch("prepare_shifted_kernel");
}

template <typename OutT>
static int match_pairs_impl(const int8_t* desc, const int32_t* norms, const int32_t* keys,
                            const int32_t* n_kpts, int n_img, int m_pad, int d,
                            const int32_t* pairs, int P, int ratio_num, int ratio_den,
                            OutT* matches0, int32_t* dist1, int32_t* dist2, void* stream) {
    SFMHIP_REQUIRE(n_img > 0 && P >= 0, "sfmhip_match_pairs: bad counts");
    SFMHIP_REQUIRE(m_pad > 0 && m_pad % kJB == 0, "sfmhip_match_pairs: m_pad must be a positive multiple of 128");
    SFMHIP_REQUIRE(ratio_num > 0 && ratio_den > 0 && ratio_num <= 65535 && ratio_den <= 65535,
                   "sfmhip_match_pairs: ratio must be a positive fraction");
    if constexpr (sizeof(OutT) == 2)
        SFMHIP_REQUIRE(m_pad <= 32767, "sfmhip_match_pairs_i16: m_pad must be <= 32767 for an int16 graph");
    if (P == 0) return SFMHIP_OK;
    SFMHIP_REQUIRE(desc && norms && keys && n_kpts && pairs && matches0,
                   "sfmhip_match_pairs: null pointer");
    const int n_iblk = ceil_div(m_pad, 256);
    const int64_t nwg64 = (int64_t)P * n_iblk;
    SFMHIP_REQUIRE(nwg64 < INT_MAX, "sfmhip_match_pairs: too many pairs for one launch");
    const int nwg = (int)nwg64;
    const long long rn2 = (long long)ratio_num * ratio_num, rd2 = (long long)ratio_den * ratio_den;
    hipStream_t s = as_stream(stream);
#define SFMHIP_LAUNCH_MATCH(DD, MF, NS, WW)                                                              \
    hipLaunchKernelGGL((match_kernel<DD, MF, NS, WW, false, OutT>), dim3(nwg), dim3(64 * WW), 0, s, desc, norms, keys, \
                       n_kpts, m_pad, pairs, n_iblk, nwg, rn2, rd2, matches0, dist1, dist2, CertArgs{})
#define SFMHIP_LAUNCH_D(DD) SFMHIP_LAUNCH_MATCH(DD, 16, 4, 4)
    switch (d) {
        case 64: SFMHIP_LAUNCH_D(64); break;
        case 128: SFMHIP_LAUNCH_D(128); break;
        case 256: SFMHIP_LAUNCH_D(256); break;
        default:
            set_error("sfmhip_match_pairs: descriptor dim %d not in {64,128,256}", d);
            return SFMHIP_E_UNSUPPORTED;
    }
#undef SFMHIP_LAUNCH_D
#undef SFMHIP_LAUNCH_MATCH
    return check_launch("match_kernel");
}

extern "C" int sfmhip_match_pairs(const int8_t* desc, const int32_t* norms, const int32_t* keys,
                                  const int32_t* n_kpts, int n_img, int m_pad, int d,
                                  const int32_t* pairs, int P, int ratio_num, int ratio_den,
                                  int32_t* matches0, int32_t* dist1, int32_t* dist2, void* stream) {
    return match_pairs_impl(desc, norms, keys, n_kpts, n_img, m_pad, d, pairs, P, ratio_num, ratio_den, matches0,
                            dist1, dist2, stream);
}

extern "C" int sfmhip_match_pairs_i16(const int8_t* desc, const int32_t* norms, const int32_t* keys,
                                      const int32_t* n_kpts, int n_img, int m_pad, int d,
                                      const int32_t* pairs, int P, int ratio_num, int ratio_den,
                                      int16_t* matches0, void* stream) {
    return match_pairs_impl(desc, norms, keys, n_kpts, n_img, m_pad, d, pairs, P, ratio_num, ratio_den, matches0,
                            (int32_t*)nullptr, (int32_t*)nullptr, stream);
}

extern "C" int sfmhip_mutual_filter(int32_t* matches0, int32_t* matches1, int P, int m_pad, void* stream) {
    SFMHIP_REQUIRE(P >= 0 && m_pad > 0, "sfmhip_mutual_filter: bad shape");
    if (P == 0) return SFMHIP_OK;
    SFMHIP_REQUIRE(matches0 && matches1, "sfmhip_mutual_filter: null pointer");
    const int64_t total = (int64_t)P * m_pad;
    const int grid = (int)std::min<int64_t>((total + 255) / 256, 8192);
    hipLaunchKernelGGL(mutual_kernel, dim3(grid), dim3(256), 0, as_stream(stream), matches0, matches1, P,
                       m_pad);
    return check_launch("mutual_kernel");
}

extern "C" int sfmhip_vq(const double* obs, int64_t n_obs, const double* code_book, int n_codes, int d,
                         int32_t* codes, double* dist, void* stream) {
    SFMHIP_REQUIRE(n_obs >= 0 && n_codes > 0 && d > 0 && d <= 256, "sfmhip_vq: bad shape (d <= 256)");
    if (n_obs == 0) return SFMHIP_OK;
    SFMHIP_REQUIRE(obs && code_book && codes && dist, "sfmhip_vq: null pointer");
    if (d == 128 && n_codes <= 256) {
        const int ncp = ceil_div(n_codes, 32) * 2;
        const size_t shm = (size_t)ncp * 4 * 2 * 64 * 16 + (size_t)ncp * 16 * sizeof(float);
        hipStream_t s = as_stream(stream);
        unsigned* amb = nullptr;
        if (scratch_alloc((void**)&amb, (size_t)(n_obs + 1) * sizeof(unsigned), s) == hipSuccess &&
            n_obs < ((int64_t)1 << 32) - 1) {
            unsigned* namb = amb + n_obs;
            (void)hipMemsetAsync(namb, 0, sizeof(unsigned), s);
            int dev = 0, n_cu = 256;
            if (hipGetDevice(&dev) == hipSuccess)
                (void)hipDeviceGetAttribute(&n_cu, hipDeviceAttributeMultiprocessorCount, dev);
            const int64_t n_wg = ((n_obs + 15) / 16 + kVqhWaves - 1) / kVqhWaves;
            auto kern = vq_f16s_kernel<0>;
            (void)hipFuncSetAttribute((const void*)kern, hipFuncAttributeMaxDynamicSharedMemorySize, (int)shm);
            hipLaunchKernelGGL(kern, dim3((unsigned)std::min<int64_t>(n_wg, n_cu)), dim3(kVqhWaves * 64), shm, s, obs,
                               n_obs, code_book, n_codes, codes, dist, amb, namb);
            int rc = check_launch("vq_f16s_kernel");
            if (rc == SFMHIP_OK) {
                hipLaunchKernelGGL(vq_exact_kernel, dim3(1024), dim3(256), 0, s, obs, code_book, n_codes, 128, amb,
                                   namb, codes, dist);
                rc = check_launch("vq_exact_kernel");
            }
            scratch_free(amb, s);
            return rc;
        }
        (void)hipGetLastError();
    }
    const int dp = d <= 32 ? 32 : d <= 64 ? 64 : d <= 128 ? 128 : 0;
    if (dp) {
        const int ld = dp + 4;
        const int max_cpp = std::min(144, (int)((150 * 1024 / 8) / (ld + 1)) / 16 * 16);
        const int passes = ceil_div(n_codes, max_cpp);
        const int cpp = ceil_div(ceil_div(n_codes, passes), 16) * 16;
        const size_t shm = (size_t)cpp * (ld + 1) * sizeof(double);
        int dev = 0, n_cu = 256;
        if (hipGetDevice(&dev) == hipSuccess) (void)hipDeviceGetAttribute(&n_cu, hipDeviceAttributeMultiprocessorCount, dev);
        const int64_t n_tiles = (n_obs + kVqmTile - 1) / kVqmTile;
        const int grid = (int)std::min<int64_t>(n_tiles, n_cu);
        hipStream_t s = as_stream(stream);
#define SFMHIP_LAUNCH_VQM(DP, FL)                                                                             \
    do {                                                                                                  \
        (void)hipFuncSetAttribute((const void*)vq_mfma_kernel<DP, FL>, hipFuncAttributeMaxDynamicSharedMemorySize, \
                                  (int)shm);                                                               \
        hipLaunchKernelGGL((vq_mfma_kernel<DP, FL>), dim3(grid), dim3(kVqmWaves * 64), shm, s, obs, n_obs,      \
                           code_book, n_codes, d, cpp, codes, dist);                                       \
    } while (0)
        if (dp == 32) SFMHIP_LAUNCH_VQM(32, false);
        else if (dp == 64) SFMHIP_LAUNCH_VQM(64, false);
        else if (d != 128) SFMHIP_LAUNCH_VQM(128, false);
        else SFMHIP_LAUNCH_VQM(128, true);
#undef SFMHIP_LAUNCH_VQM
        return check_launch("vq_mfma_kernel");
    }
    const int64_t blocks = (n_obs + kVqObsPerBlock - 1) / kVqObsPerBlock;
    SFMHIP_REQUIRE(blocks < INT_MAX, "sfmhip_vq: too many observations");
    const size_t shm = (size_t)(kVqObsPerBlock * d + kVqCodesPerChunk * (d + 1)) * sizeof(double);
    SFMHIP_REQUIRE(shm <= 160 * 1024, "sfmhip_vq: descriptor dim too large for the LDS tiles");
    hipLaunchKernelGGL(vq_kernel, dim3((int)blocks), dim3(256), shm, as_stream(stream), obs, n_obs, code_book,
                       n_codes, d, codes, dist);
    return check_launch("vq_kernel");
}

extern "C" int sfmhip_desc_residual(const float* desc_f, const int8_t* desc_q, int n_img, int m_pad, int d,
                                    const int32_t* n_kpts, int mode, double* resid_row, double* resid_img,
                                    void* stream) {
    SFMHIP_REQUIRE(desc_f && desc_q && n_kpts && resid_row && resid_img, "sfmhip_desc_residual: null pointer");
    SFMHIP_REQUIRE(n_img > 0 && m_pad > 0 && d > 0, "sfmhip_desc_residual: bad shape");
    SFMHIP_REQUIRE(mode == 0 || mode == 1, "sfmhip_desc_residual: mode must be 0 or 1");
    const int64_t rows = (int64_t)n_img * m_pad;
    SFMHIP_REQUIRE(rows < INT_MAX, "sfmhip_desc_residual: too many rows");
    hipStream_t s = as_stream(stream);
    if (hipMemsetAsync(resid_img, 0, (size_t)n_img * sizeof(double), s) != hipSuccess) return check_launch("memset");
    hipLaunchKernelGGL(desc_residual_kernel, dim3(ceil_div(rows, 4)), dim3(256), 0, s, desc_f, desc_q, (int)rows, m_pad,
                       d, n_kpts, mode, resid_row, reinterpret_cast<unsigned long long*>(resid_img));
    return check_launch("desc_residual_kernel");
}

template <typename OutT>
static int match_exact_impl(const int8_t* desc, const int32_t* norms, const int32_t* keys,
                            const int8_t* desc_q, const float* desc_f, const double* resid_row,
                            const double* resid_img, int mode, const int32_t* n_kpts, int n_img,
                            int m_pad, int d, const int32_t* pairs, int P, int ratio_num, int ratio_den,
                            OutT* matches0, int32_t* dist1, int32_t* dist2, uint32_t* n_resolved,
                            void* stream, const uint8_t* dense = nullptr, const int32_t* h_bank = nullptr,
                            const float* hf_bank = nullptr) {
    const bool fp6 = dense && knobs().match_fp6 != 0;
    if (dense) {
        SFMHIP_REQUIRE(mode == 1 && !dist1 && !dist2 && (d == 128 || d == 256),
                       "sfmhip_match_pairs_exact_fp6: float mode, d in {128,256}, no distance outputs");
    }
    SFMHIP_REQUIRE(n_img > 0 && P >= 0, "sfmhip_match_pairs_exact: bad counts");
    SFMHIP_REQUIRE(m_pad > 0 && m_pad % kJB == 0, "sfmhip_match_pairs_exact: m_pad must be a positive multiple of 128");
    SFMHIP_REQUIRE(mode == 0 || mode == 1, "sfmhip_match_pairs_exact: mode must be 0 or 1");
    SFMHIP_REQUIRE(ratio_num > 0 && ratio_den > 0 && ratio_num <= 65535 && ratio_den <= 65535,
                   "sfmhip_match_pairs_exact: ratio must be a positive fraction");
    if constexpr (sizeof(OutT) == 2)
        SFMHIP_REQUIRE(m_pad <= 32767, "sfmhip_match_pairs_exact_i16: m_pad must be <= 32767 for an int16 graph");
    if (P == 0) return SFMHIP_OK;
    SFMHIP_REQUIRE(desc && norms && keys && desc_q && desc_f && resid_row && resid_img && n_kpts && pairs && matches0,
                   "sfmhip_match_pairs_exact: null pointer");
    const int IB = fp6 ? 16 * kFp6Tiles * kFp6Waves : 256;
    const int n_iblk = ceil_div(m_pad, IB);
    const int64_t nwg64 = (int64_t)P * n_iblk;
    SFMHIP_REQUIRE(nwg64 < INT_MAX, "sfmhip_match_pairs_exact: too many pairs for one launch");
    const int nwg = (int)nwg64;
    const long long rn2 = (long long)ratio_num * ratio_num, rd2 = (long long)ratio_den * ratio_den;
    const CertArgs ca{resid_row, resid_img, mode == 0 ? 1.0 : 1.0 / 127.0, knobs().match_cert == 0 ? 1 : 0};
    hipStream_t s = as_stream(stream);
    int dev = 0, n_cu = 256;
    if (hipGetDevice(&dev) == hipSuccess) (void)hipDeviceGetAttribute(&n_cu, hipDeviceAttributeMultiprocessorCount, dev);
    const int64_t nchunk = ((int64_t)P * m_pad + 63) / 64;
    const int rgrid = (int)std::min<int64_t>((nchunk + 3) / 4, (int64_t)n_cu * 8);
    if (n_resolved && hipMemsetAsync(n_resolved, 0, sizeof(uint32_t), s) != hipSuccess) return check_launch("memset");
    const int64_t total = (int64_t)P * m_pad;
    void* rbuf = nullptr;
    const size_t rlist_bytes = (size_t)n_img * kResolveBucket * sizeof(int64_t);
    const size_t rcnt_bytes = ((size_t)n_img + 1) * sizeof(unsigned);
    const size_t roff_bytes = (3 * (size_t)n_img + 33) * sizeof(unsigned);
    const size_t ritem_bytes = 3 * (size_t)n_img * (kResolveBucket / kResolveRows + 1) * sizeof(int);
    const bool value_only = !dist1 && !dist2;
    const size_t rbytes = 2 * rlist_bytes + rcnt_bytes + roff_bytes + ritem_bytes;
    const size_t hn = value_only && !h_bank ? (size_t)n_img * m_pad : 0;
    if (scratch_alloc(&rbuf, rbytes + hn * (fp6 ? 2 : 1) * sizeof(int32_t), s) != hipSuccess) {
        (void)hipGetLastError();
        set_error("sfmhip_match_pairs_exact: scratch allocation failed");
        return SFMHIP_E_HIP;
    }
    int64_t* rlist = reinterpret_cast<int64_t*>(rbuf);
    unsigned* rcnt = reinterpret_cast<unsigned*>(static_cast<char*>(rbuf) + rlist_bytes);
    unsigned* rflag = rcnt + n_img;
    int64_t* rflat = reinterpret_cast<int64_t*>(static_cast<char*>(rbuf) + rlist_bytes + rcnt_bytes + roff_bytes);
    unsigned* roff = reinterpret_cast<unsigned*>(static_cast<char*>(rbuf) + rlist_bytes + rcnt_bytes);
    unsigned* rokey = roff + n_img;
    int* roimg = reinterpret_cast<int*>(rokey + n_img + 1);
    unsigned* rxr = reinterpret_cast<unsigned*>(roimg + n_img);
    unsigned* rir = rxr + 16;
    int* ritems = reinterpret_cast<int*>(static_cast<char*>(rbuf) + 2 * rlist_bytes + rcnt_bytes + roff_bytes);
    if (hipMemsetAsync(rcnt, 0, rcnt_bytes, s) != hipSuccess) {
        scratch_free(rbuf, s);
        return check_launch("memset");
    }
    const int rxgrid = n_cu * 2;
    const float* hf = hf_bank;
    if (h_bank) keys = h_bank;
    if (hn) {
        int32_t* h = reinterpret_cast<int32_t*>(static_cast<char*>(rbuf) + rbytes);
        float* hf_call = fp6 ? reinterpret_cast<float*>(h + hn) : nullptr;
        hipLaunchKernelGGL(key_values_kernel, dim3(std::min(ceil_div((int64_t)hn, 256), 4096)), dim3(256), 0, s, keys,
                           (int64_t)hn, h, hf_call);
        keys = h;
        hf = hf_call;
    }
#define SFMHIP_LAUNCH_EXACT(DD)                                                                                  \
    if (fp6) {                                                                                                    \
        if constexpr (DD % 128 == 0)                                                                              \
            hipLaunchKernelGGL((match_fp6_kernel<DD, OutT>), dim3(nwg), dim3(64 * kFp6Waves), 0, s, dense, desc, norms,  \
                               keys, hf, n_kpts, m_pad, pairs, n_iblk, nwg, rn2, rd2, matches0, ca);              \
    } else if (value_only) {                                                                                             \
        hipLaunchKernelGGL((match_kernel<DD, 16, 4, 4, true, OutT, kValueOnlyTiles>), dim3(nwg), dim3(256), 0, s, desc, \
                           norms, keys, n_kpts, m_pad, pairs, n_iblk, nwg, rn2, rd2, matches0, dist1, dist2, ca);  \
    } else {                                                                                                      \
        hipLaunchKernelGGL((match_kernel<DD, 16, 4, 4, true, OutT>), dim3(nwg), dim3(256), 0, s, desc, norms, keys, \
                           n_kpts, m_pad, pairs, n_iblk, nwg, rn2, rd2, matches0, dist1, dist2, ca);              \
    }                                                                                                             \
    if (int rc = check_launch("match_kernel<cert>")) {                                                          \
        scratch_free(rbuf, s);                                                                                    \
        return rc;                                                                                                \
    }                                                                                                             \
    hipLaunchKernelGGL(resolve_collect_kernel<OutT>, dim3(rgrid), dim3(256), 0, s, matches0, total, m_pad, pairs, rcnt,  \
                       rlist, rflag);                                                                             \
    hipLaunchKernelGGL(resolve_offsets_kernel, dim3(1), dim3(1024), 0, s, rcnt, n_img, roff, rokey, roimg, rxr,      \
                       ritems, rir, rflag);                                                                       \
    hipLaunchKernelGGL(resolve_flatten_kernel, dim3(n_cu), dim3(256), 0, s, rokey, roimg, n_img, rlist, rflat,     \
                       rflag);                                                                                    \
    hipLaunchKernelGGL((match_resolve_batched_kernel<DD, OutT>), dim3(rxgrid), dim3(256), 0, s, desc, norms, desc_f, n_kpts,  \
                       m_pad, pairs, n_img, resid_row, resid_img, mode == 0 ? 1.0 : 127.0, (double)rn2,          \
                       (double)rd2, matches0, n_resolved, rflat, ritems, rir, rflag);                              \
    hipLaunchKernelGGL((match_resolve_kernel<DD, OutT>), dim3(rgrid), dim3(256), 0, s, desc_q, desc_f, n_kpts, m_pad,   \
                       pairs, P, resid_row, resid_img, mode == 0 ? 1.0 : 127.0, (double)rn2, (double)rd2,        \
                       matches0, n_resolved, rflag)
    switch (d) {
        case 64: SFMHIP_LAUNCH_EXACT(64); break;
        case 128: SFMHIP_LAUNCH_EXACT(128); break;
        case 256: SFMHIP_LAUNCH_EXACT(256); break;
        default:
            set_error("sfmhip_match_pairs_exact: descriptor dim %d not in {64,128,256}", d);
            scratch_free(rbuf, s);
            return SFMHIP_E_UNSUPPORTED;
    }
#undef SFMHIP_LAUNCH_EXACT
    const int rc = check_launch("match_resolve_kernel");
    scratch_free(rbuf, s);
    return rc;
}

extern "C" int sfmhip_match_pairs_exact(const int8_t* desc, const int32_t* norms, const int32_t* keys,
                                        const int8_t* desc_q, const float* desc_f, const double* resid_row,
                                        const double* resid_img, int mode, const int32_t* n_kpts, int n_img,
                                        int m_pad, int d, const int32_t* pairs, int P, int ratio_num, int ratio_den,
                                        int32_t* matches0, int32_t* dist1, int32_t* dist2, uint32_t* n_resolved,
                                        void* stream) {
    return match_exact_impl(desc, norms, keys, desc_q, desc_f, resid_row, resid_img, mode, n_kpts, n_img, m_pad, d,
                            pairs, P, ratio_num, ratio_den, matches0, dist1, dist2, n_resolved, stream);
}

extern "C" int sfmhip_match_pairs_exact_i16(const int8_t* desc, const int32_t* norms, const int32_t* keys,
                                            const int8_t* desc_q, const float* desc_f, const double* resid_row,
                                            const double* resid_img, int mode, const int32_t* n_kpts, int n_img,
                                            int m_pad, int d, const int32_t* pairs, int P, int ratio_num,
                                            int ratio_den, int16_t* matches0, uint32_t* n_resolved, void* stream) {
    return match_exact_impl(desc, norms, keys, desc_q, desc_f, resid_row, resid_img, mode, n_kpts, n_img, m_pad, d,
                            pairs, P, ratio_num, ratio_den, matches0, (int32_t*)nullptr, (int32_t*)nullptr,
                            n_resolved, stream);
}

extern "C" int sfmhip_match_pairs_exact_fp6(const uint8_t* dense, const int8_t* g, const int32_t* norms,
                                            const int32_t* keys, const float* desc_f, const double* resid_row,
                                            const double* resid_img, const int32_t* n_kpts, int n_img, int m_pad,
                                            int d, const int32_t* pairs, int P, int ratio_num, int ratio_den,
                                            int32_t* matches0, uint32_t* n_resolved, void* stream) {
    SFMHIP_REQUIRE(dense || P == 0, "sfmhip_match_pairs_exact_fp6: null pointer");
    return match_exact_impl(g, norms, keys, g, desc_f, resid_row, resid_img, 1, n_kpts, n_img, m_pad, d, pairs, P,
                            ratio_num, ratio_den, matches0, (int32_t*)nullptr, (int32_t*)nullptr, n_resolved, stream,
                            dense);
}

extern "C" int sfmhip_match_pairs_exact_fp6_i16(const uint8_t* dense, const int8_t* g, const int32_t* norms,
                                                const int32_t* keys, const float* desc_f, const double* resid_row,
                                                const double* resid_img, const int32_t* n_kpts, int n_img, int m_pad,
                                                int d, const int32_t* pairs, int P, int ratio_num, int ratio_den,
                                                int16_t* matches0, uint32_t* n_resolved, void* stream) {
    SFMHIP_REQUIRE(dense || P == 0, "sfmhip_match_pairs_exact_fp6_i16: null pointer");
    return match_exact_impl(g, norms, keys, g, desc_f, resid_row, resid_img, 1, n_kpts, n_img, m_pad, d, pairs, P,
                            ratio_num, ratio_den, matches0, (int32_t*)nullptr, (int32_t*)nullptr, n_resolved, stream,
                            dense);
}

extern "C" int sfmhip_match_key_values(const int32_t* keys, int n_img, int m_pad, int32_t* h, float* hf, void* stream) {
    SFMHIP_REQUIRE(keys && h && hf, "sfmhip_match_key_values: null pointer");
    SFMHIP_REQUIRE(n_img > 0 && m_pad > 0, "sfmhip_match_key_values: bad shape");
    const int64_t n = (int64_t)n_img * m_pad;
    hipLaunchKernelGGL(key_values_kernel, dim3(std::min(ceil_div(n, 256), 4096)), dim3(256), 0, as_stream(stream), keys, n,
                       h, hf);
    return check_launch("key_values_kernel");
}

extern "C" int sfmhip_match_pairs_exact_fp6_kv(const uint8_t* dense, const int8_t* g, const int32_t* norms,
                                               const int32_t* h, const float* hf, const float* desc_f,
                                               const double* resid_row, const double* resid_img, const int32_t* n_kpts,
                                               int n_img, int m_pad, int d, const int32_t* pairs, int P, int ratio_num,
                                               int ratio_den, int32_t* matches0, uint32_t* n_resolved, void* stream) {
    SFMHIP_REQUIRE((dense && hf) || P == 0, "sfmhip_match_pairs_exact_fp6_kv: null pointer");
    return match_exact_impl(g, norms, h, g, desc_f, resid_row, resid_img, 1, n_kpts, n_img, m_pad, d, pairs, P,
                            ratio_num, ratio_den, matches0, (int32_t*)nullptr, (int32_t*)nullptr, n_resolved, stream,
                            dense, h, hf);
}

extern "C" int sfmhip_match_pairs_exact_fp6_kv_i16(const uint8_t* dense, const int8_t* g, const int32_t* norms,
                                                   const int32_t* h, const float* hf, const float* desc_f,
                                                   const double* resid_row, const double* resid_img,
                                                   const int32_t* n_kpts, int n_img, int m_pad, int d,
                                                   const int32_t* pairs, int P, int ratio_num, int ratio_den,
                                                   int16_t* matches0, uint32_t* n_resolved, void* stream) {
    SFMHIP_REQUIRE((dense && hf) || P == 0, "sfmhip_match_pairs_exact_fp6_kv_i16: null pointer");
    return match_exact_impl(g, norms, h, g, desc_f, resid_row, resid_img, 1, n_kpts, n_img, m_pad, d, pairs, P,
                            ratio_num, ratio_den, matches0, (int32_t*)nullptr, (int32_t*)nullptr, n_resolved, stream,
                            dense, h, hf);
}
```

Before: 685,100 pairs/s.

## Append undecided rows from match kernel and restructure exact resolve pipeline

The value-only match tail now appends undecided rows directly into per-image buckets using a wave-aggregated atomic, which removes the separate full scan of the match output plus the offsets and flatten kernels in the value-only path. The resolve stage is split into an int8 MFMA prefilter kernel that is sliced per image, a per-row resolve kernel, and an 'every' fallback kernel. Threshold data (tq, qrow) is precomputed at append time. In exchange this adds global atomics inside the hot match kernel, extra scratch buffers, a reset kernel, and fixed capacity limits that fall back to the slow resolve path when exceeded.

Result: no change. 690,700 pairs/s (median of 6 runs) (+0.8%).

```diff
diff --git a/3d_reconstruction_amd/csrc/match.hip b/3d_reconstruction_amd/csrc/match.hip
--- a/3d_reconstruction_amd/csrc/match.hip
+++ b/3d_reconstruction_amd/csrc/match.hip
@@ -194,11 +194,26 @@
     __device__ static int row(int q, int grp) { return 4 * grp + q; }
 };
 
+constexpr int kResolveBucket = 4096;
+constexpr int kResolveRowsMax = 1 << 16;
+constexpr int kResolveEveryMax = 1024;
+enum { kHeadFlag = 0, kHeadRows = 1, kHeadEvery = 2, kHeadCnt = 3 };
+struct ResolveRows {
+    unsigned* head;
+    unsigned* bucket;
+    int64_t* entry;
+    int64_t* qrow;
+    double* tq;
+    double s;
+    template <typename OutT>
+    __device__ __forceinline__ void put(unsigned t, unsigned slot, int b, int64_t e, int64_t arow, int mark, double E) const;
+};
 struct CertArgs {
     const double* erow;
     const double* eimg;
     double inv_s;
     int force;
+    ResolveRows rr;
 };
 constexpr int kUndecidedBase = -3;
 constexpr int kValueOnlyTiles = 4;
@@ -218,6 +233,37 @@
 __device__ __forceinline__ double mark_sqrt_d2(int mark) {
     if constexpr (sizeof(OutT) == 2) return (double)(kUndecidedBase - mark) * 0.125;
     else return sqrt((double)(kUndecidedBase - mark));
+}
+
+template <typename OutT>
+__device__ __forceinline__ void ResolveRows::put(unsigned t, unsigned slot, int b, int64_t e, int64_t arow, int mark,
+                                                 double E) const {
+    if (t < (unsigned)kResolveRowsMax && slot < (unsigned)kResolveBucket) {
+        const size_t at = (size_t)b * kResolveBucket + slot;
+        const double se = E * s * (1.0 + 1e-12);
+        const double bq = (se + (mark_sqrt_d2<OutT>(mark) + se) * (1.0 + 1e-12)) * (1.0 + 1e-12);
+        entry[t] = e;
+        bucket[at] = t;
+        qrow[at] = arow;
+        tq[at] = floor(bq * bq) + 1.0;
+    } else {
+        atomicOr(head + kHeadFlag, 1u);
+    }
+}
+template <typename OutT>
+__device__ __forceinline__ void resolve_append(const ResolveRows& rr, bool und, int64_t e, int64_t arow, int b, int mark,
+                                               double E, int lane) {
+    const unsigned long long bal = __ballot(und);
+    if (bal == 0) return;
+    const int n = __popcll(bal), leader = __builtin_ctzll(bal);
+    unsigned t0 = 0, s0 = 0;
+    if (lane == leader) {
+        t0 = atomicAdd(rr.head + kHeadRows, (unsigned)n);
+        s0 = atomicAdd(rr.head + kHeadCnt + b, (unsigned)n);
+    }
+    const unsigned k = (unsigned)__popcll(bal & ((1ull << lane) - 1ull));
+    const unsigned t = __shfl(t0, leader) + k, slot = __shfl(s0, leader) + k;
+    if (und) rr.template put<OutT>(t, slot, b, e, arow, mark, E);
 }
 
 __device__ __forceinline__ int certify(int d1lo, int d1hi, int d2lo, int d2hi, double E, double inv_s, double rn2,
@@ -238,9 +284,9 @@
 __device__ __forceinline__ void value_only_tail(const int (&w1)[NS], const int (&w2)[NS], const int (&wr)[NS],
                                                 const int8_t* __restrict__ desc, const int8_t* __restrict__ bdesc,
                                                 const int32_t* __restrict__ bkeys, const int32_t* __restrict__ norms,
-                                                int a, int b, int m_pad, int na_rows, int ibase, int grp, int lr,
-                                                int lane, long long rn2, long long rd2, OutT* __restrict__ out_m,
-                                                const CertArgs& ca) {
+                                                int pair, int a, int b, int m_pad, int na_rows, int ibase, int grp,
+                                                int lr, int lane, long long rn2, long long rd2,
+                                                OutT* __restrict__ out_m, const CertArgs& ca) {
     constexpr int NG = 64 / MF;
     int v1 = INT_MIN, v2 = INT_MIN, loc = 0;
 #pragma unroll
@@ -315,6 +361,7 @@
         res = v == 0 ? -1 : (v > 0 && hidx >= 0) ? hidx : undecided_mark<OutT>(du2);
     }
     if (i < m_pad) out_m[i] = (OutT)res;
+    resolve_append<OutT>(ca.rr, res <= kUndecidedBase, (int64_t)pair * m_pad + i, (int64_t)a * m_pad + i, b, res, E, lane);
 }
 
 template <int D, int MF, int NS, int WAVES, bool CERT = false, typename OutT = int32_t, int VG = 0>
@@ -479,8 +526,8 @@
     }
 
     if constexpr (VO) {
-        value_only_tail<D, MF, NS, VG, OutT>(w1, w2, wr, desc, bdesc, bkeys, norms, a, b, m_pad, na_rows, ibase, grp, lr,
-                                             lane, rn2, rd2, out_m, ca);
+        value_only_tail<D, MF, NS, VG, OutT>(w1, w2, wr, desc, bdesc, bkeys, norms, pair, a, b, m_pad, na_rows, ibase, grp,
+                                             lr, lane, rn2, rd2, out_m, ca);
         return;
     }
     if constexpr (D <= 128) {
@@ -786,8 +833,8 @@
             v2[s] = (int)(64.f * w2[4 * q + s]);
             vr[s] = wr[4 * q + s];
         }
-        value_only_tail<D, MF, 4, VG, OutT>(v1, v2, vr, g, g + (size_t)b * m_pad * D, h + (size_t)b * m_pad, norms, a, b,
-                                            m_pad, na_rows, ibase + q * 4 * MF, grp, lr, lane, rn2, rd2, out_m, ca);
+        value_only_tail<D, MF, 4, VG, OutT>(v1, v2, vr, g, g + (size_t)b * m_pad * D, h + (size_t)b * m_pad, norms, pair, a,
+                                            b, m_pad, na_rows, ibase + q * 4 * MF, grp, lr, lane, rn2, rd2, out_m, ca);
     }
 }
 
@@ -1392,285 +1439,278 @@
     }
 }
 
-constexpr int kResolveBucket = 4096;
+
+__global__ void resolve_reset_kernel(unsigned* __restrict__ z, int n, unsigned* __restrict__ n_resolved) {
+    const int t = blockIdx.x * blockDim.x + threadIdx.x;
+    if (t < n) z[t] = 0u;
+    if (t == 0 && n_resolved) *n_resolved = 0u;
+}
+
 template <typename OutT>
 __global__ __launch_bounds__(256) void resolve_collect_kernel(const OutT* __restrict__ m0, int64_t total, int m_pad,
                                                               const int32_t* __restrict__ pairs,
-                                                              unsigned* __restrict__ cnt, int64_t* __restrict__ list,
-                                                              unsigned* __restrict__ overflow) {
-    auto take = [&](int64_t e) {
-        const int b = pairs[2 * (int)(e / m_pad) + 1];
-        const unsigned slot = atomicAdd(cnt + b, 1u);
-        if (slot < (unsigned)kResolveBucket) list[(size_t)b * kResolveBucket + slot] = e;
-        else atomicOr(overflow, 1u);
-    };
+                                                              const double* __restrict__ erow,
+                                                              const double* __restrict__ eimg, ResolveRows rr) {
     constexpr int PER = 16 / sizeof(OutT);
     const int64_t n4 = total / PER;
     const int4* m4 = reinterpret_cast<const int4*>(m0);
     for (int64_t e4 = (int64_t)blockIdx.x * blockDim.x + threadIdx.x; e4 < n4; e4 += (int64_t)gridDim.x * blockDim.x) {
         const int4 v = m4[e4];
-        if constexpr (sizeof(OutT) == 2) {
-            const unsigned w[4] = {(unsigned)v.x, (unsigned)v.y, (unsigned)v.z, (unsigned)v.w};
-            bool any = false;
-#pragma unroll
-            for (int h = 0; h < 4; ++h) {
-                any |= (short)(w[h] & 0xFFFFu) <= kUndecidedBase;
-                any |= (short)(w[h] >> 16) <= kUndecidedBase;
-            }
-            if (!any) continue;
-#pragma unroll
-            for (int h = 0; h < 4; ++h) {
-                if ((short)(w[h] & 0xFFFFu) <= kUndecidedBase) take(PER * e4 + 2 * h);
-                if ((short)(w[h] >> 16) <= kUndecidedBase) take(PER * e4 + 2 * h + 1);
-            }
-        } else {
-            if (min(min(v.x, v.y), min(v.z, v.w)) > kUndecidedBase) continue;
-            if (v.x <= kUndecidedBase) take(4 * e4);
-            if (v.y <= kUndecidedBase) take(4 * e4 + 1);
-            if (v.z <= kUndecidedBase) take(4 * e4 + 2);
-            if (v.w <= kUndecidedBase) take(4 * e4 + 3);
+        const OutT* w = reinterpret_cast<const OutT*>(&v);
+#pragma unroll
+        for (int h = 0; h < PER; ++h) {
+            if ((int)w[h] > kUndecidedBase) continue;
+            const int64_t e = PER * e4 + h;
+            const int pair = (int)(e / m_pad), b = pairs[2 * pair + 1];
+            const int64_t arow = (int64_t)pairs[2 * pair] * m_pad + (int)(e % m_pad);
+            const unsigned t = atomicAdd(rr.head + kHeadRows, 1u), slot = atomicAdd(rr.head + kHeadCnt + b, 1u);
+            rr.template put<OutT>(t, slot, b, e, arow, (int)w[h], erow[arow] + eimg[b]);
         }
     }
 }
 
 constexpr int kResolveRows = 16;
-__global__ __launch_bounds__(1024) void resolve_offsets_kernel(
-    const unsigned* __restrict__ cnt, int n_img, unsigned* __restrict__ off,
-    unsigned* __restrict__ okey , int* __restrict__ oimg,
-    unsigned* __restrict__ xr, int* __restrict__ items ,
-    unsigned* __restrict__ ir , const unsigned* __restrict__ overflow) {
-    __shared__ unsigned sr[1024], sk[1024];
-    __shared__ unsigned sxs[9], sks[9];
-    if (*overflow != 0u) return;
-    const int tid = threadIdx.x;
-    const int cap = n_img * (kResolveBucket / kResolveRows + 1);
-    int ps[9];
-    ps[0] = 0;
-#pragma unroll
-    for (int x = 0; x < 8; ++x) ps[x + 1] = ps[x] + (x < n_img ? (n_img - x + 7) / 8 : 0);
-    unsigned carry_r = 0, carry_k = 0;
-    for (int base = 0; base < n_img; base += 1024) {
-        const int p = base + tid;
-        int b = -1;
-        unsigned cb = 0, ni = 0;
-        if (p < n_img) {
-            int x = 0;
-#pragma unroll
-            for (int y = 1; y < 8; ++y) x += (p >= ps[y]) ? 1 : 0;
-            b = x + 8 * (p - ps[x]);
-            cb = min(cnt[b], (unsigned)kResolveBucket);
-            ni = (cb + kResolveRows - 1) / kResolveRows;
-        }
-        sr[tid] = cb;
-        sk[tid] = ni;
+constexpr int kPrefTiles = 4;
+template <int D, typename OutT>
+__global__ __launch_bounds__(256) void match_resolve_prefilter_kernel(
+    const int8_t* __restrict__ q , const int32_t* __restrict__ norms,
+    const int32_t* __restrict__ nk, int m_pad, ResolveRows rr, int nslab, int tps ,
+    unsigned* __restrict__ ccnt, int* __restrict__ cand) {
+    using M16 = Mfma<16>;
+    constexpr int W4 = D / 4, R = kResolveRows, TW = kPrefTiles, KK = D / M16::KB;
+    __shared__ __attribute__((aligned(16))) int sqa[R][W4];
+    __shared__ int snq[R];
+    if (rr.head[kHeadFlag] != 0u) return;
+    const int b = blockIdx.x / nslab, slab = blockIdx.x % nslab;
+    const int nrows = (int)min(rr.head[kHeadCnt + b], (unsigned)kResolveBucket);
+    const int nb = nk[b];
+    const int t0 = slab * tps, t1 = min(t0 + tps, (nb + 15) / 16);
+    if (nrows == 0 || t0 >= t1) return;
+    const int tid = threadIdx.x, lane = tid & 63, wave = tid >> 6;
+    const int lr = lane & 15, grp = lane >> 4;
+    const size_t bbase = (size_t)b * m_pad;
+    const unsigned* bucket = rr.bucket + (size_t)b * kResolveBucket;
+    const int64_t* qrow = rr.qrow + (size_t)b * kResolveBucket;
+    const double* tq = rr.tq + (size_t)b * kResolveBucket;
+    i32x4 av[TW][KK], nv[TW];
+#pragma unroll
+    for (int k = 0; k < TW; ++k) {
+        const int j0 = 16 * min(t0 + wave + 4 * k, t1 - 1);
+        const int8_t* rp = q + (bbase + j0 + lr) * D + grp * 16;
+#pragma unroll
+        for (int kk = 0; kk < KK; ++kk) av[k][kk] = *reinterpret_cast<const i32x4*>(rp + kk * M16::KB);
+        nv[k] = *reinterpret_cast<const i32x4*>(norms + bbase + j0 + 4 * grp);
+    }
+    for (int r0 = 0; r0 < nrows; r0 += R) {
+        const int nr = min(R, nrows - r0);
         __syncthreads();
-        for (int d = 1; d < 1024; d <<= 1) {
-            const unsigned vr = tid >= d ? sr[tid - d] : 0u, vk = tid >= d ? sk[tid - d] : 0u;
-            __syncthreads();
-            sr[tid] += vr;
-            sk[tid] += vk;
-            __syncthreads();
-        }
-        const unsigned run = carry_r + sr[tid] - cb, k0 = carry_k + sk[tid] - ni;
-        if (b >= 0) {
-            off[b] = run;
-            okey[p] = run;
-            oimg[p] = b;
-#pragma unroll
-            for (int x = 0; x < 8; ++x)
-                if (p == ps[x]) {
-                    sxs[x] = run;
-                    sks[x] = k0;
-                }
-            for (unsigned i = 0; i < ni; ++i) {
-                items[k0 + i] = (int)(run + i * kResolveRows);
-                items[cap + k0 + i] = (int)min((unsigned)kResolveRows, cb - i * kResolveRows);
-                items[2 * cap + k0 + i] = b;
-            }
-        }
-        carry_r += sr[1023];
-        carry_k += sk[1023];
-        __syncthreads();
-    }
-    if (tid < 9) {
-        if (tid == 8 || ps[tid] >= n_img) {
-            sxs[tid] = carry_r;
-            sks[tid] = carry_k;
-        }
-    }
-    __syncthreads();
-    if (tid < 8) {
-        xr[tid] = sxs[tid];
-        xr[8 + tid] = sxs[tid + 1] - sxs[tid];
-        ir[tid] = sks[tid];
-        ir[8 + tid] = sks[tid + 1] - sks[tid];
-    }
-    if (tid == 0) okey[n_img] = carry_r;
-}
-__global__ __launch_bounds__(256) void resolve_flatten_kernel(const unsigned* __restrict__ okey,
-                                                              const int* __restrict__ oimg, int n_img,
-                                                              const int64_t* __restrict__ list,
-                                                              int64_t* __restrict__ flat,
-                                                              const unsigned* __restrict__ overflow) {
-    if (*overflow != 0u) return;
-    const unsigned total = okey[n_img];
-    for (unsigned t = blockIdx.x * blockDim.x + threadIdx.x; t < total; t += gridDim.x * blockDim.x) {
-        int lo = 0, hi = n_img - 1;
-        while (lo < hi) {
-            const int mid = (lo + hi + 1) >> 1;
-            if (okey[mid] <= t) lo = mid;
-            else hi = mid - 1;
-        }
-        flat[t] = list[(size_t)oimg[lo] * kResolveBucket + (t - okey[lo])];
-    }
-}
-
-template <int D, typename OutT>
-__global__ __launch_bounds__(256) void match_resolve_batched_kernel(
-    const int8_t* __restrict__ q , const int32_t* __restrict__ norms,
-    const float* __restrict__ x, const int32_t* __restrict__ nk, int m_pad,
-    const int32_t* __restrict__ pairs, int n_img, const double* __restrict__ erow, const double* __restrict__ eimg,
-    double s, double rn2, double rd2, OutT* __restrict__ m0, unsigned* __restrict__ n_resolved,
-    const int64_t* __restrict__ flat, const int* __restrict__ items, const unsigned* __restrict__ ir,
-    const unsigned* __restrict__ overflow) {
-    constexpr int W4 = D / 4, R = kResolveRows;
-    __shared__ __attribute__((aligned(16))) int sqa[R][W4];
-    __shared__ float sxa[R][D];
-    __shared__ int scand[R][kResolveCap];
-    __shared__ int sncand[R], sna[R], sccd[R];
-    __shared__ double stq[R];
-    __shared__ int64_t se_[R];
-    if (*overflow != 0u) return;
-    const int tid = threadIdx.x, lane = tid & 63, wave = tid >> 6;
-    const int cap = n_img * (kResolveBucket / kResolveRows + 1);
-    const int xcd = blockIdx.x % 8, nx = (gridDim.x + 7 - xcd) / 8;
-    const unsigned ib = ir[xcd], in = ir[8 + xcd];
-    for (unsigned k = blockIdx.x / 8; k < in; k += nx) {
-        const int f0 = items[ib + k], nr = items[cap + ib + k], b = items[2 * cap + ib + k];
-        const int nb = nk[b];
         for (int t = tid; t < nr * W4; t += 256) {
             const int r = t / W4, w = t % W4;
-            const int64_t e = flat[f0 + r];
-            const size_t arow = (size_t)pairs[2 * (int)(e / m_pad)] * m_pad + (int)(e % m_pad);
-            sqa[r][w] = reinterpret_cast<const int*>(q + arow * D)[w];
-        }
-        for (int t = tid; t < nr * D; t += 256) {
-            const int r = t / D, kk = t % D;
-            const int64_t e = flat[f0 + r];
-            const size_t arow = (size_t)pairs[2 * (int)(e / m_pad)] * m_pad + (int)(e % m_pad);
-            sxa[r][kk] = x[arow * D + kk];
-        }
-        if (tid < R) sncand[tid] = 0;
+            sqa[r][w] = reinterpret_cast<const int*>(q + (size_t)qrow[r0 + r] * D)[w];
+        }
+        const bool live = lr < nr;
+        const double tq_r = live ? tq[r0 + lr] : -1.0;
+        const unsigned flat = live ? bucket[r0 + lr] : 0u;
+        const int nrm_r = live ? norms[qrow[r0 + lr]] : 0;
         __syncthreads();
         for (int r = wave; r < nr; r += 4) {
             int na = 0;
             for (int w = lane; w < W4; w += 64) na = __builtin_amdgcn_sdot4(sqa[r][w], sqa[r][w], na, false);
 #pragma unroll
             for (int off = 32; off >= 1; off >>= 1) na += __shfl_xor(na, off);
-            if (lane == 0) {
-                const int64_t e = flat[f0 + r];
-                const size_t arow = (size_t)pairs[2 * (int)(e / m_pad)] * m_pad + (int)(e % m_pad);
-                const double se = (erow[arow] + eimg[b]) * s * (1.0 + 1e-12);
-                const double bq = (se + (mark_sqrt_d2<OutT>((int)m0[e]) + se) * (1.0 + 1e-12)) * (1.0 + 1e-12);
-                stq[r] = floor(bq * bq) + 1.0;
-                sna[r] = na;
-                sccd[r] = norms[arow] - na;
-                se_[r] = e;
-            }
+            if (lane == 0) snq[r] = na;
         }
         __syncthreads();
-        {
-            using M16 = Mfma<16>;
-            constexpr int KK = D / M16::KB;
-            const int lr = lane & 15, grp = lane >> 4;
-            i32x4 bqv[KK];
-#pragma unroll
-            for (int kk = 0; kk < KK; ++kk) bqv[kk] = *reinterpret_cast<const i32x4*>(&sqa[lr][kk * 16 + grp * 4]);
-            const bool live = lr < nr;
-            const long long na_r = live ? (long long)sna[lr] - sccd[lr] : 0;
-            const double tq_r = live ? stq[lr] : -1.0;
-            const size_t bbase = (size_t)b * m_pad;
-            constexpr int TG = 4;
-            for (int jg = wave * 16; jg < nb; jg += 64 * TG) {
-                i32x4 av[TG][KK], nv[TG];
-#pragma unroll
-                for (int t = 0; t < TG; ++t) {
-                    const int j0 = min(jg + 64 * t, m_pad - 16);
-                    const int8_t* rp = q + (bbase + j0 + lr) * D + grp * 16;
-#pragma unroll
-                    for (int kk = 0; kk < KK; ++kk) av[t][kk] = *reinterpret_cast<const i32x4*>(rp + kk * M16::KB);
-                    nv[t] = *reinterpret_cast<const i32x4*>(norms + bbase + j0 + 4 * grp);
+        i32x4 bqv[KK];
+#pragma unroll
+        for (int kk = 0; kk < KK; ++kk) bqv[kk] = *reinterpret_cast<const i32x4*>(&sqa[lr][kk * 16 + grp * 4]);
+        const long long na_r = live ? 2LL * snq[lr] - nrm_r : 0;
+#pragma unroll
+        for (int k = 0; k < TW; ++k) {
+            const int t = t0 + wave + 4 * k;
+            if (t >= t1) continue;
+            i32x4 acc = {0, 0, 0, 0};
+#pragma unroll
+            for (int kk = 0; kk < KK; ++kk) acc = M16::run(av[k][kk], bqv[kk], acc);
+#pragma unroll
+            for (int e = 0; e < 4; ++e) {
+                const int j = 16 * t + 4 * grp + e;
+                if (live && j < nb && (double)(na_r + nv[k][e] - 2LL * acc[e]) <= tq_r) {
+                    const unsigned pos = atomicAdd(ccnt + flat, 1u);
+                    if (pos < (unsigned)kResolveCap) cand[(size_t)flat * kResolveCap + pos] = j;
                 }
-#pragma unroll
-                for (int t = 0; t < TG; ++t) {
-                    const int j0 = jg + 64 * t;
-                    i32x4 acc = {0, 0, 0, 0};
-#pragma unroll
-                    for (int kk = 0; kk < KK; ++kk) acc = M16::run(av[t][kk], bqv[kk], acc);
-#pragma unroll
-                    for (int e = 0; e < 4; ++e) {
-                        const int j = j0 + 4 * grp + e;
-                        if (live && j < nb && (double)(na_r + nv[t][e] - 2LL * acc[e]) <= tq_r) {
-                            const int pos = atomicAdd(&sncand[lr], 1);
-                            if (pos < kResolveCap) scand[lr][pos] = j;
-                        }
-                    }
-                }
-            }
-        }
-        __syncthreads();
-        for (int r = wave; r < nr; r += 4) {
-            const int ncand = sncand[r];
-            const bool every = ncand > kResolveCap;
+            }
+        }
+    }
+}
+
+template <int D, typename OutT>
+__global__ __launch_bounds__(256) void match_resolve_rows_kernel(
+    const float* __restrict__ x, const int32_t* __restrict__ nk, int m_pad, const int32_t* __restrict__ pairs,
+    double rn2, double rd2, OutT* __restrict__ m0, unsigned* __restrict__ n_resolved, ResolveRows rr,
+    const unsigned* __restrict__ ccnt, const int* __restrict__ cand, unsigned* __restrict__ elist) {
+    __shared__ float sxa_[4][D];
+    if (rr.head[kHeadFlag] != 0u) return;
+    const int lane = threadIdx.x & 63, wave = threadIdx.x >> 6;
+    float* sxa = sxa_[wave];
+    const unsigned total = rr.head[kHeadRows];
+    for (unsigned t = blockIdx.x * 4 + wave; t < total; t += gridDim.x * 4) {
+        const int64_t e = rr.entry[t];
+        const int pair = (int)(e / m_pad);
+        const int a = pairs[2 * pair], b = pairs[2 * pair + 1], nb = nk[b];
+        const size_t arow = (size_t)a * m_pad + (int)(e % m_pad);
+        for (int k = lane; k < D; k += 64) sxa[k] = x[arow * D + k];
+        __builtin_amdgcn_fence(__ATOMIC_RELEASE, "wavefront");
+        __builtin_amdgcn_wave_barrier();
+        __builtin_amdgcn_fence(__ATOMIC_ACQUIRE, "wavefront");
+        const int ncand = (int)min(ccnt[t], (unsigned)INT_MAX);
+        const bool every = ncand > kResolveCap;
 #ifdef SFMHIP_RESOLVE_PROF
-            if (lane == 0) {
-                atomicAdd(&g_rprof[0], 1ull);
-                atomicAdd(&g_rprof[1], (unsigned long long)ncand);
-                if (every) atomicAdd(&g_rprof[2], 1ull);
-                atomicMax(&g_rprof[3], (unsigned long long)ncand);
-                atomicAdd(&g_rprof[4 + min(ncand / 64, 11)], 1ull);
-            }
+        if (lane == 0) {
+            atomicAdd(&g_rprof[0], 1ull);
+            atomicAdd(&g_rprof[1], (unsigned long long)ncand);
+            if (every) atomicAdd(&g_rprof[2], 1ull);
+            atomicMax(&g_rprof[3], (unsigned long long)ncand);
+            atomicAdd(&g_rprof[4 + min(ncand / 64, 11)], 1ull);
+        }
 #endif
-            const int nc = every ? nb : ncand;
-            double v1 = __builtin_inf(), v2 = __builtin_inf();
-            int j1 = INT_MAX;
-            for (int t = lane; t < nc; t += 64) {
-                const int j = every ? t : scand[r][t];
-                const float4* xb = reinterpret_cast<const float4*>(x + ((size_t)b * m_pad + j) * D);
-                double acc = 0.0;
-                for (int k4 = 0; k4 < D / 4; ++k4) {
-                    const float4 xv = xb[k4];
-                    double df;
-                    df = (double)sxa[r][4 * k4] - (double)xv.x;
-                    acc = acc + df * df;
-                    df = (double)sxa[r][4 * k4 + 1] - (double)xv.y;
-                    acc = acc + df * df;
-                    df = (double)sxa[r][4 * k4 + 2] - (double)xv.z;
-                    acc = acc + df * df;
-                    df = (double)sxa[r][4 * k4 + 3] - (double)xv.w;
-                    acc = acc + df * df;
-                }
-                if (acc < v1 || (acc == v1 && j < j1)) { v2 = v1; v1 = acc; j1 = j; }
-                else if (acc < v2) v2 = acc;
-            }
-#pragma unroll
-            for (int off = 32; off >= 1; off >>= 1) {
-                const double o1 = __shfl_xor(v1, off), o2 = __shfl_xor(v2, off);
-                const int oj = __shfl_xor(j1, off);
-                const bool mine = v1 < o1 || (v1 == o1 && j1 < oj);
-                const double n2 = mine ? fmin(v2, o1) : fmin(o2, v1);
-                if (!mine) { v1 = o1; j1 = oj; }
-                v2 = n2;
-            }
-            const double p1 = rd2 * v1, e1 = __builtin_fma(rd2, v1, -p1);
-            const double p2 = rn2 * v2, e2 = __builtin_fma(rn2, v2, -p2);
-            const bool acc_ok = p1 < p2 || (p1 == p2 && e1 < e2);
-            if (lane == 0) {
-                m0[se_[r]] = (OutT)(acc_ok ? j1 : -1);
-                if (n_resolved) atomicAdd(n_resolved, 1u);
-            }
-        }
-        __syncthreads();
+        if (every) {
+            unsigned k = 0;
+            if (lane == 0) k = atomicAdd(rr.head + kHeadEvery, 1u);
+            k = __shfl(k, 0);
+            if (k < (unsigned)kResolveEveryMax) {
+                if (lane == 0) elist[k] = t;
+                continue;
+            }
+        }
+        const int nc = every ? nb : ncand;
+        const int* scand = cand + (size_t)t * kResolveCap;
+        double v1 = __builtin_inf(), v2 = __builtin_inf();
+        int j1 = INT_MAX;
+        for (int c = lane; c < nc; c += 64) {
+            const int j = every ? c : scand[c];
+            const float4* xb = reinterpret_cast<const float4*>(x + ((size_t)b * m_pad + j) * D);
+            double acc = 0.0;
+#pragma unroll 8
+            for (int k4 = 0; k4 < D / 4; ++k4) {
+                const float4 xv = xb[k4];
+                double df;
+                df = (double)sxa[4 * k4] - (double)xv.x;
+                acc = acc + df * df;
+                df = (double)sxa[4 * k4 + 1] - (double)xv.y;
+                acc = acc + df * df;
+                df = (double)sxa[4 * k4 + 2] - (double)xv.z;
+                acc = acc + df * df;
+                df = (double)sxa[4 * k4 + 3] - (double)xv.w;
+                acc = acc + df * df;
+            }
+            if (acc < v1 || (acc == v1 && j < j1)) { v2 = v1; v1 = acc; j1 = j; }
+            else if (acc < v2) v2 = acc;
+        }
+#pragma unroll
+        for (int off = 32; off >= 1; off >>= 1) {
+            const double o1 = __shfl_xor(v1, off), o2 = __shfl_xor(v2, off);
+            const int oj = __shfl_xor(j1, off);
+            const bool mine = v1 < o1 || (v1 == o1 && j1 < oj);
+            const double n2 = mine ? fmin(v2, o1) : fmin(o2, v1);
+            if (!mine) { v1 = o1; j1 = oj; }
+            v2 = n2;
+        }
+        const double p1 = rd2 * v1, e1 = __builtin_fma(rd2, v1, -p1);
+        const double p2 = rn2 * v2, e2 = __builtin_fma(rn2, v2, -p2);
+        const bool acc_ok = p1 < p2 || (p1 == p2 && e1 < e2);
+        if (lane == 0) {
+            m0[e] = (OutT)(acc_ok ? j1 : -1);
+            if (n_resolved) atomicAdd(n_resolved, 1u);
+        }
+        __builtin_amdgcn_wave_barrier();
+    }
+}
+
+template <int D, typename OutT>
+__global__ __launch_bounds__(256) void match_resolve_every_kernel(
+    const float* __restrict__ x, const int32_t* __restrict__ nk, int m_pad, const int32_t* __restrict__ pairs,
+    double rn2, double rd2, OutT* __restrict__ m0, unsigned* __restrict__ n_resolved, ResolveRows rr,
+    const unsigned* __restrict__ elist, unsigned* __restrict__ edone, double* part ) {
+    __shared__ float sxa_[4][D];
+    if (rr.head[kHeadFlag] != 0u) return;
+    const int lane = threadIdx.x & 63, wave = threadIdx.x >> 6;
+    float* sxa = sxa_[wave];
+    const unsigned n_every = min(rr.head[kHeadEvery], (unsigned)kResolveEveryMax);
+    const unsigned cpr = (unsigned)m_pad / 64u;
+    auto merge = [](double& v1, double& v2, int& j1, double o1, double o2, int oj) {
+        const bool mine = v1 < o1 || (v1 == o1 && j1 < oj);
+        const double n2 = mine ? fmin(v2, o1) : fmin(o2, v1);
+        if (!mine) { v1 = o1; j1 = oj; }
+        v2 = n2;
+    };
+    for (unsigned u = blockIdx.x * 4 + wave; u < n_every * cpr; u += gridDim.x * 4) {
+        const unsigned k = u / cpr, c = u % cpr;
+        const int64_t e = rr.entry[elist[k]];
+        const int pair = (int)(e / m_pad);
+        const int a = pairs[2 * pair], b = pairs[2 * pair + 1], nb = nk[b];
+        const unsigned nchunk = ((unsigned)nb + 63u) / 64u;
+        if (c >= nchunk) continue;
+        const size_t arow = (size_t)a * m_pad + (int)(e % m_pad);
+        for (int kk = lane; kk < D; kk += 64) sxa[kk] = x[arow * D + kk];
+        __builtin_amdgcn_fence(__ATOMIC_RELEASE, "wavefront");
+        __builtin_amdgcn_wave_barrier();
+        __builtin_amdgcn_fence(__ATOMIC_ACQUIRE, "wavefront");
+        double v1 = __builtin_inf(), v2 = __builtin_inf();
+        int j1 = INT_MAX;
+        const int j = (int)c * 64 + lane;
+        if (j < nb) {
+            const float4* xb = reinterpret_cast<const float4*>(x + ((size_t)b * m_pad + j) * D);
+            double acc = 0.0;
+#pragma unroll 8
+            for (int k4 = 0; k4 < D / 4; ++k4) {
+                const float4 xv = xb[k4];
+                double df;
+                df = (double)sxa[4 * k4] - (double)xv.x;
+                acc = acc + df * df;
+                df = (double)sxa[4 * k4 + 1] - (double)xv.y;
+                acc = acc + df * df;
+                df = (double)sxa[4 * k4 + 2] - (double)xv.z;
+                acc = acc + df * df;
+                df = (double)sxa[4 * k4 + 3] - (double)xv.w;
+                acc = acc + df * df;
+            }
+            v1 = acc;
+            j1 = j;
+        }
+#pragma unroll
+        for (int off = 32; off >= 1; off >>= 1) merge(v1, v2, j1, __shfl_xor(v1, off), __shfl_xor(v2, off), __shfl_xor(j1, off));
+        double* pr = part + ((size_t)k * cpr + c) * 3;
+        unsigned old = 0;
+        if (lane == 0) {
+            __hip_atomic_store(pr, v1, __ATOMIC_RELAXED, __HIP_MEMORY_SCOPE_AGENT);
+            __hip_atomic_store(pr + 1, v2, __ATOMIC_RELAXED, __HIP_MEMORY_SCOPE_AGENT);
+            __hip_atomic_store(pr + 2, (double)j1, __ATOMIC_RELAXED, __HIP_MEMORY_SCOPE_AGENT);
+            __threadfence();
+            old = atomicAdd(edone + k, 1u);
+        }
+        old = __shfl(old, 0);
+        __builtin_amdgcn_wave_barrier();
+        if (old != nchunk - 1) continue;
+        __threadfence();
+        v1 = v2 = __builtin_inf();
+        j1 = INT_MAX;
+        for (unsigned cc = lane; cc < nchunk; cc += 64) {
+            const double* po = part + ((size_t)k * cpr + cc) * 3;
+            const double o1 = __hip_atomic_load(po, __ATOMIC_RELAXED, __HIP_MEMORY_SCOPE_AGENT);
+            const double o2 = __hip_atomic_load(po + 1, __ATOMIC_RELAXED, __HIP_MEMORY_SCOPE_AGENT);
+            const int oj = (int)__hip_atomic_load(po + 2, __ATOMIC_RELAXED, __HIP_MEMORY_SCOPE_AGENT);
+            merge(v1, v2, j1, o1, o2, oj);
+        }
+#pragma unroll
+        for (int off = 32; off >= 1; off >>= 1) merge(v1, v2, j1, __shfl_xor(v1, off), __shfl_xor(v2, off), __shfl_xor(j1, off));
+        const double p1 = rd2 * v1, e1 = __builtin_fma(rd2, v1, -p1);
+        const double p2 = rn2 * v2, e2 = __builtin_fma(rn2, v2, -p2);
+        const bool acc_ok = p1 < p2 || (p1 == p2 && e1 < e2);
+        if (lane == 0) {
+            m0[e] = (OutT)(acc_ok ? j1 : -1);
+            if (n_resolved) atomicAdd(n_resolved, 1u);
+        }
     }
 }
 
@@ -1949,52 +1989,56 @@
     SFMHIP_REQUIRE(nwg64 < INT_MAX, "sfmhip_match_pairs_exact: too many pairs for one launch");
     const int nwg = (int)nwg64;
     const long long rn2 = (long long)ratio_num * ratio_num, rd2 = (long long)ratio_den * ratio_den;
-    const CertArgs ca{resid_row, resid_img, mode == 0 ? 1.0 : 1.0 / 127.0, knobs().match_cert == 0 ? 1 : 0};
     hipStream_t s = as_stream(stream);
     int dev = 0, n_cu = 256;
     if (hipGetDevice(&dev) == hipSuccess) (void)hipDeviceGetAttribute(&n_cu, hipDeviceAttributeMultiprocessorCount, dev);
     const int64_t nchunk = ((int64_t)P * m_pad + 63) / 64;
     const int rgrid = (int)std::min<int64_t>((nchunk + 3) / 4, (int64_t)n_cu * 8);
-    if (n_resolved && hipMemsetAsync(n_resolved, 0, sizeof(uint32_t), s) != hipSuccess) return check_launch("memset");
     const int64_t total = (int64_t)P * m_pad;
+    const int ntile = m_pad / 16;
+    const int nslab = std::max(8, ceil_div(ntile, 4 * kPrefTiles)), tps = ceil_div(ntile, nslab);
+    SFMHIP_REQUIRE((int64_t)n_img * nslab < INT_MAX, "sfmhip_match_pairs_exact: too many images for one launch");
     void* rbuf = nullptr;
-    const size_t rlist_bytes = (size_t)n_img * kResolveBucket * sizeof(int64_t);
-    const size_t rcnt_bytes = ((size_t)n_img + 1) * sizeof(unsigned);
-    const size_t roff_bytes = (3 * (size_t)n_img + 33) * sizeof(unsigned);
-    const size_t ritem_bytes = 3 * (size_t)n_img * (kResolveBucket / kResolveRows + 1) * sizeof(int);
+    const size_t entry_bytes = (size_t)kResolveRowsMax * sizeof(int64_t);
+    const size_t part_bytes = (size_t)kResolveEveryMax * (m_pad / 64) * 3 * sizeof(double);
+    const size_t elist_bytes = (size_t)kResolveEveryMax * sizeof(unsigned);
+    const size_t cand_bytes = (size_t)kResolveRowsMax * kResolveCap * sizeof(int);
+    const size_t bucket_bytes = (size_t)n_img * kResolveBucket * sizeof(unsigned);
+    const int n_zero = kHeadCnt + n_img + kResolveRowsMax + kResolveEveryMax;
     const bool value_only = !dist1 && !dist2;
-    const size_t rbytes = 2 * rlist_bytes + rcnt_bytes + roff_bytes + ritem_bytes;
+    const size_t slot8_bytes = (size_t)n_img * kResolveBucket * 8;
+    const size_t front_bytes = entry_bytes + part_bytes + 2 * slot8_bytes + elist_bytes + cand_bytes;
+    const size_t rbytes = front_bytes + bucket_bytes + (size_t)n_zero * sizeof(unsigned);
     const size_t hn = value_only && !h_bank ? (size_t)n_img * m_pad : 0;
     if (scratch_alloc(&rbuf, rbytes + hn * (fp6 ? 2 : 1) * sizeof(int32_t), s) != hipSuccess) {
         (void)hipGetLastError();
         set_error("sfmhip_match_pairs_exact: scratch allocation failed");
         return SFMHIP_E_HIP;
     }
-    int64_t* rlist = reinterpret_cast<int64_t*>(rbuf);
-    unsigned* rcnt = reinterpret_cast<unsigned*>(static_cast<char*>(rbuf) + rlist_bytes);
-    unsigned* rflag = rcnt + n_img;
-    int64_t* rflat = reinterpret_cast<int64_t*>(static_cast<char*>(rbuf) + rlist_bytes + rcnt_bytes + roff_bytes);
-    unsigned* roff = reinterpret_cast<unsigned*>(static_cast<char*>(rbuf) + rlist_bytes + rcnt_bytes);
-    unsigned* rokey = roff + n_img;
-    int* roimg = reinterpret_cast<int*>(rokey + n_img + 1);
-    unsigned* rxr = reinterpret_cast<unsigned*>(roimg + n_img);
-    unsigned* rir = rxr + 16;
-    int* ritems = reinterpret_cast<int*>(static_cast<char*>(rbuf) + 2 * rlist_bytes + rcnt_bytes + roff_bytes);
-    if (hipMemsetAsync(rcnt, 0, rcnt_bytes, s) != hipSuccess) {
-        scratch_free(rbuf, s);
-        return check_launch("memset");
-    }
-    const int rxgrid = n_cu * 2;
+    char* rp = static_cast<char*>(rbuf);
+    double* rpart = reinterpret_cast<double*>(rp + entry_bytes);
+    int64_t* rqrow = reinterpret_cast<int64_t*>(rp + entry_bytes + part_bytes);
+    double* rtq = reinterpret_cast<double*>(rp + entry_bytes + part_bytes + slot8_bytes);
+    unsigned* relist = reinterpret_cast<unsigned*>(rp + entry_bytes + part_bytes + 2 * slot8_bytes);
+    int* rcand = reinterpret_cast<int*>(rp + entry_bytes + part_bytes + 2 * slot8_bytes + elist_bytes);
+    unsigned* rhead = reinterpret_cast<unsigned*>(rp + front_bytes + bucket_bytes);
+    unsigned* rccnt = rhead + kHeadCnt + n_img;
+    unsigned* redone = rccnt + kResolveRowsMax;
+    const ResolveRows rr{rhead, reinterpret_cast<unsigned*>(rp + front_bytes), reinterpret_cast<int64_t*>(rp), rqrow, rtq,
+                         mode == 0 ? 1.0 : 127.0};
+    const CertArgs ca{resid_row, resid_img, mode == 0 ? 1.0 : 1.0 / 127.0, knobs().match_cert == 0 ? 1 : 0, rr};
+    hipLaunchKernelGGL(resolve_reset_kernel, dim3(ceil_div(n_zero, 256)), dim3(256), 0, s, rhead, n_zero, n_resolved);
     const float* hf = hf_bank;
     if (h_bank) keys = h_bank;
     if (hn) {
-        int32_t* h = reinterpret_cast<int32_t*>(static_cast<char*>(rbuf) + rbytes);
+        int32_t* h = reinterpret_cast<int32_t*>(rp + rbytes);
         float* hf_call = fp6 ? reinterpret_cast<float*>(h + hn) : nullptr;
         hipLaunchKernelGGL(key_values_kernel, dim3(std::min(ceil_div((int64_t)hn, 256), 4096)), dim3(256), 0, s, keys,
                            (int64_t)hn, h, hf_call);
         keys = h;
         hf = hf_call;
     }
+    const double rs = mode == 0 ? 1.0 : 127.0;
 #define SFMHIP_LAUNCH_EXACT(DD)                                                                                  \
     if (fp6) {                                                                                                    \
         if constexpr (DD % 128 == 0)                                                                              \
@@ -2011,18 +2055,18 @@
         scratch_free(rbuf, s);                                                                                    \
         return rc;                                                                                                \
     }                                                                                                             \
-    hipLaunchKernelGGL(resolve_collect_kernel<OutT>, dim3(rgrid), dim3(256), 0, s, matches0, total, m_pad, pairs, rcnt,  \
-                       rlist, rflag);                                                                             \
-    hipLaunchKernelGGL(resolve_offsets_kernel, dim3(1), dim3(1024), 0, s, rcnt, n_img, roff, rokey, roimg, rxr,      \
-                       ritems, rir, rflag);                                                                       \
-    hipLaunchKernelGGL(resolve_flatten_kernel, dim3(n_cu), dim3(256), 0, s, rokey, roimg, n_img, rlist, rflat,     \
-                       rflag);                                                                                    \
-    hipLaunchKernelGGL((match_resolve_batched_kernel<DD, OutT>), dim3(rxgrid), dim3(256), 0, s, desc, norms, desc_f, n_kpts,  \
-                       m_pad, pairs, n_img, resid_row, resid_img, mode == 0 ? 1.0 : 127.0, (double)rn2,          \
-                       (double)rd2, matches0, n_resolved, rflat, ritems, rir, rflag);                              \
+    if (!value_only)                                     \
+        hipLaunchKernelGGL(resolve_collect_kernel<OutT>, dim3(rgrid), dim3(256), 0, s, matches0, total, m_pad, pairs, \
+                           resid_row, resid_img, rr);                                                             \
+    hipLaunchKernelGGL((match_resolve_prefilter_kernel<DD, OutT>), dim3(n_img * nslab), dim3(256), 0, s, desc, norms,  \
+                       n_kpts, m_pad, rr, nslab, tps, rccnt, rcand);                                              \
+    hipLaunchKernelGGL((match_resolve_rows_kernel<DD, OutT>), dim3(n_cu * 8), dim3(256), 0, s, desc_f, n_kpts, m_pad, \
+                       pairs, (double)rn2, (double)rd2, matches0, n_resolved, rr, rccnt, rcand, relist);          \
+    hipLaunchKernelGGL((match_resolve_every_kernel<DD, OutT>), dim3(n_cu * 4), dim3(256), 0, s, desc_f, n_kpts, m_pad, \
+                       pairs, (double)rn2, (double)rd2, matches0, n_resolved, rr, relist, redone, rpart);         \
     hipLaunchKernelGGL((match_resolve_kernel<DD, OutT>), dim3(rgrid), dim3(256), 0, s, desc_q, desc_f, n_kpts, m_pad,   \
-                       pairs, P, resid_row, resid_img, mode == 0 ? 1.0 : 127.0, (double)rn2, (double)rd2,        \
-                       matches0, n_resolved, rflag)
+                       pairs, P, resid_row, resid_img, rs, (double)rn2, (double)rd2, matches0, n_resolved,        \
+                       rhead + kHeadFlag)
     switch (d) {
         case 64: SFMHIP_LAUNCH_EXACT(64); break;
         case 128: SFMHIP_LAUNCH_EXACT(128); break;
```
